# Algolzw/image-restoration-sde

Hardware: AMD Instinct MI355X
Metric: restored images/sec at 256x256, 100-step IR-SDE reverse sampler (higher is better)
Workload: dtype f32; 1 GPU; IR-SDE deraining ConditionalUNet nf=64 depth=4, reverse_sde, batch=16/GPU 256x256, T=100 (BASELINE.json configs[1]); compute_dtype=fp32, global_batch=16

## Files before the change

### image_restoration_sde_amd/_lib.py

```python
import ctypes
import os
import subprocess
import threading

_HERE = os.path.dirname(os.path.abspath(__file__))
LIB_PATH = os.environ.get("IRSDE_LIB_PATH") or os.path.join(_HERE, "libirsde_hip.so")
CSRC = os.path.join(_HERE, "csrc")

MODE = {"sde": 0, "ode": 1, "posterior": 2, "dsde_sde": 3, "dsde_ode": 4}
COEF_STRIDE = 12
FLAG_KEEP_ACTIVATIONS = 1
FLAG_NAIVE_CONV = 2
FLAG_NO_WINOGRAD = 4
FLAG_NO_WINOGRAD_F43 = 8
FLAG_UNCOND_FULLATTN = 16
FLAG_BF16 = 32
FLAG_NAF_INTRO_SKIP = 64
FLAG_BF16_ACT = 128
FLAG_NO_FUSED_LN = 256
FLAG_NAF_LENS = 512
FLAG_FP16 = 1024
FLAG_NO_WINOGRAD_FUSED = 2048
FLAG_NO_FUSED_ATTN = 4096
FLAG_NO_NAF_CHAIN = 8192
FLAG_SPLIT_BF16X2 = 16384
FLAG_SPLIT_F16X2 = 32768
FLAG_NAF_STEREO = 65536
FLAG_NAF_UNCOND = 131072
SAMPLE_GRAPH = 1
SAMPLE_PROFILE = 2

SYMBOLS = [
    "irsde_last_error", "irsde_version", "irsde_create", "irsde_create_nafnet", "irsde_destroy", "irsde_num_weights",
    "irsde_weight_name", "irsde_weight_shape", "irsde_load_weight", "irsde_finalize_weights",
    "irsde_set_schedule", "irsde_unet_forward", "irsde_sample", "irsde_sde_step", "irsde_philox_normal",
    "irsde_get_profile", "irsde_debug_tap", "irsde_work_model", "irsde_debug_conv", "irsde_plan_describe", "irsde_bench_conv", "irsde_op_profile", "irsde_debug_split_gemm", "irsde_bench_naf_chain", "irsde_debug_force_subbatches", "irsde_debug_force_chain_groups", "irsde_debug_scam",
    "irsde_eval_metrics", "irsde_tensor2img",
    "irsde_set_lens_info", "irsde_create_latent_unet", "irsde_latent_shapes", "irsde_latent_encode", "irsde_latent_decode", "irsde_latent_hidden",
]


class IrsdeLibraryError(RuntimeError):
    pass


class IrsdeError(RuntimeError):
    pass


class Config(ctypes.Structure):
    _fields_ = [("in_nc", ctypes.c_int32), ("out_nc", ctypes.c_int32), ("nf", ctypes.c_int32),
                ("depth", ctypes.c_int32), ("device", ctypes.c_int32), ("flags", ctypes.c_int32)]


class NafConfig(ctypes.Structure):
    _fields_ = [("img_channel", ctypes.c_int32), ("width", ctypes.c_int32), ("middle_blk_num", ctypes.c_int32),
                ("n_enc", ctypes.c_int32), ("enc_blk_nums", ctypes.c_int32 * 8), ("n_dec", ctypes.c_int32),
                ("dec_blk_nums", ctypes.c_int32 * 8), ("device", ctypes.c_int32), ("flags", ctypes.c_int32)]


class LatentConfig(ctypes.Structure):
    _fields_ = [("in_ch", ctypes.c_int32), ("out_ch", ctypes.c_int32), ("ch", ctypes.c_int32), ("n_mult", ctypes.c_int32),
                ("ch_mult", ctypes.c_int32 * 8), ("embed_dim", ctypes.c_int32), ("device", ctypes.c_int32),
                ("flags", ctypes.c_int32)]


_lib = None
_lock = threading.Lock()


PROBES_LIB_PATH = os.path.join(_HERE, "libirsde_hip_probes.so")


def build_library(force=False, verbose=False, probes=True):
    if force:
        subprocess.run(["make", "-C", CSRC, "clean"], check=True, capture_output=not verbose)
    for extra in ([], ["PROBES=1"]) if probes else ([],):
        r = subprocess.run(["make", "-j8", "-C", CSRC] + extra, capture_output=True, text=True)
        if r.returncode != 0:
            raise IrsdeLibraryError("building libirsde_hip%s.so failed:\n" % ("_probes" if extra else "") + r.stdout + r.stderr)
        if verbose:
            print(r.stdout)
    return LIB_PATH


def _declare(lib):
    c = ctypes
    P = c.c_void_p
    lib.irsde_last_error.restype = c.c_char_p
    lib.irsde_last_error.argtypes = []
    lib.irsde_version.restype = c.c_int
    lib.irsde_create.argtypes = [c.POINTER(Config), c.POINTER(P)]
    lib.irsde_create_nafnet.argtypes = [c.POINTER(NafConfig), c.POINTER(P)]
    lib.irsde_destroy.argtypes = [P]
    lib.irsde_destroy.restype = None
    lib.irsde_num_weights.argtypes = [P]
    lib.irsde_weight_name.argtypes = [P, c.c_int]
    lib.irsde_weight_name.restype = c.c_char_p
    lib.irsde_weight_shape.argtypes = [P, c.c_int, c.POINTER(c.c_int64), c.POINTER(c.c_int)]
    lib.irsde_load_weight.argtypes = [P, c.c_char_p, P, c.POINTER(c.c_int64), c.c_int]
    lib.irsde_finalize_weights.argtypes = [P]
    lib.irsde_set_schedule.argtypes = [P, c.c_int, P]
    lib.irsde_unet_forward.argtypes = [P, P, P, c.POINTER(c.c_int64), c.c_int, c.c_int, c.c_int, c.c_int, P, P]
    lib.irsde_sample.argtypes = [P, c.c_int, P, P, P, c.c_uint64, c.c_uint64, c.c_int, c.c_int, c.c_int,
                                 c.c_int, c.c_int, P, P, c.c_int]
    lib.irsde_sde_step.argtypes = [c.c_int, c.c_int, P, P, P, P, P, c.c_uint64, c.c_uint64, c.c_int, c.c_int,
                                   c.c_int, c.c_int, P]
    lib.irsde_philox_normal.argtypes = [P, c.c_int, c.c_int, c.c_int, c.c_uint64, c.c_uint64, P]
    lib.irsde_get_profile.argtypes = [P, c.POINTER(c.c_double)]
    lib.irsde_debug_tap.argtypes = [P, c.c_char_p, P, c.POINTER(c.c_int64)]
    lib.irsde_work_model.argtypes = [P, c.c_int, c.c_int, c.c_int, c.POINTER(c.c_double)]
    lib.irsde_debug_conv.argtypes = [P, c.c_int, P, c.c_int, c.c_int, c.c_int, c.c_int, c.c_int, P, c.c_int, c.c_int,
                                     c.c_int, c.c_int, c.c_int, P, P, c.c_int, c.c_int, P, P, c.c_int, c.c_int, P]
    lib.irsde_plan_describe.argtypes = [P, c.c_int, c.c_int, c.c_int, c.c_char_p, c.c_int]
    lib.irsde_op_profile.argtypes = [P, c.c_char_p, c.c_int]
    lib.irsde_bench_conv.argtypes = [c.c_int] * 11 + [c.POINTER(c.c_double)]
    lib.irsde_bench_naf_chain.argtypes = [c.c_int] * 4 + [c.POINTER(c.c_double)]
    lib.irsde_debug_force_subbatches.argtypes = [c.c_int]
    lib.irsde_debug_force_chain_groups.argtypes = [c.c_int]
    lib.irsde_debug_scam.argtypes = [P, c.c_int, c.c_int, c.c_int, c.c_int] + [P] * 12 + [P, P]
    lib.irsde_debug_split_gemm.argtypes = [P, P, P, c.c_int, c.c_int, c.c_int, c.c_int, c.c_int, P]
    lib.irsde_eval_metrics.argtypes = [P, P, c.c_int, c.c_int, c.c_int, c.c_int, c.c_int, c.POINTER(c.c_double), P]
    lib.irsde_tensor2img.argtypes = [P, P, c.c_int, c.c_int, c.c_int, c.c_int, P]
    lib.irsde_set_lens_info.argtypes = [P, c.POINTER(c.c_float), c.c_int]
    lib.irsde_create_latent_unet.argtypes = [c.POINTER(LatentConfig), c.POINTER(P)]
    lib.irsde_latent_shapes.argtypes = [P, c.c_int, c.c_int, c.POINTER(c.c_int64), c.POINTER(c.c_int64), c.POINTER(c.c_int)]
    lib.irsde_latent_encode.argtypes = [P, P, c.c_int, c.c_int, c.c_int, P, c.POINTER(P), P]
    lib.irsde_latent_decode.argtypes = [P, P, c.POINTER(P), c.c_int, c.c_int, c.c_int, P, P]
    lib.irsde_latent_hidden.argtypes = [P, c.c_int, c.c_int, c.c_int, c.c_int, P, P]
    for name in SYMBOLS:
        getattr(lib, name)
    return lib


def lib():
    global _lib
    with _lock:
        if _lib is None:
            if not os.path.exists(LIB_PATH):
                raise IrsdeLibraryError(
                    "libirsde_hip.so not found at %s — build it with `python -c 'import __graft_entry__ as g; "
                    "g.build()'` or `make -C %s`. There is no CPU/PyTorch fallback for this path." % (LIB_PATH, CSRC))
            try:
                _lib = _declare(ctypes.CDLL(LIB_PATH))
            except OSError as ex:
                raise IrsdeLibraryError("failed to load %s: %s" % (LIB_PATH, ex)) from ex
        return _lib


_probes = None


def probes_lib():
    global _probes
    with _lock:
        if _probes is None:
            if not os.path.exists(PROBES_LIB_PATH):
                raise IrsdeLibraryError("libirsde_hip_probes.so not found at %s — build it with `make -C %s PROBES=1`" % (PROBES_LIB_PATH, CSRC))
            try:
                _probes = _declare(ctypes.CDLL(PROBES_LIB_PATH))
            except OSError as ex:
                raise IrsdeLibraryError("failed to load %s: %s" % (PROBES_LIB_PATH, ex)) from ex
        return _probes


def check(rc, L=None):
    if rc != 0:
        msg = (L or lib()).irsde_last_error()
        raise IrsdeError("libirsde_hip error %d: %s" % (rc, msg.decode() if msg else "?"))


def stream_ptr(torch_stream=None):
    import torch
    s = torch_stream if torch_stream is not None else torch.cuda.current_stream()
    return ctypes.c_void_p(s.cuda_stream)
```

### image_restoration_sde_amd/csrc/common.h

```cpp
#pragma once
#include <hip/hip_runtime.h>
#include <cstdint>
#include <cstdio>
#include <cstdlib>
#include <stdexcept>
#include <string>
#include <vector>

namespace irsde {

struct HipError : std::runtime_error {
    using std::runtime_error::runtime_error;
};
struct HipOutOfMemory : HipError {
    using HipError::HipError;
};

inline int tuning_env_int(const char* name, int dflt) {
    static const bool on = [] { const char* t = getenv("IRSDE_TUNING"); return t && atoi(t) == 1; }();
    if (!on) return dflt;
    const char* v = getenv(name);
    return v ? atoi(v) : dflt;
}

// ... 50 lines not shown
    const float* in0 = nullptr;
    const float* in1 = nullptr;
    int C0 = 0, C1 = 0, Hin = 0, Win = 0, in_shift = 0;
    int B = 0, TH = 0, TW = 0, T = 0;
    int tile = 2;
    float* V = nullptr;
    unsigned short* Vs = nullptr;
    int nplanes = 0;
    long long v_plane = 0;
    int v_f16 = 0;
    float v_scale = 1.f;
    int v_pairs = 0;
    const float* M = nullptr;
    int Cout = 0;
    float* out = nullptr;
    int out_stride = 0;
    const float* bias = nullptr;
    const float* film = nullptr;
    int film_bstride = 0;
    int silu = 0;
    const float* res = nullptr;
    int res_stride = 0;
};
void launch_wino_input(const WinoParams& p, hipStream_t s);
struct SplitGemmArgs {
    const unsigned short* a = nullptr;
    const unsigned short* b = nullptr;
    float* out = nullptr;
    long long plA = 0, plB = 0, pA = 0, pB = 0, pO = 0;
    int M = 0, N = 0, K = 0, lda = 0, ldc = 0;
    float out_scale = 1.f;
    int n_inner = 1;
    int nblk_n = 0;
};
void gemm_split_global_init();
int gemm_split_inner(int M, int N, int ncomp);
void launch_gemm_split_pairs(const SplitGemmArgs& a, int ncomp, hipStream_t s, int abl = 0, bool f16 = false);
void launch_split_pairs(const float* in, unsigned short* out, size_t rows, int K, hipStream_t s, bool f16 = false,
                        float scale = 1.0f);
void launch_gemm_split(const SplitGemmArgs& a, int nplanes, int ncomp, hipStream_t s);
void launch_split_planes(const float* in, unsigned short* out, size_t n, size_t plane, int nplanes, hipStream_t s, bool f16 = false,
                         float scale = 1.0f);
void launch_wino_output(const WinoParams& p, hipStream_t s);
void wino_transform_weights(const float* w_packed, int Cout, int Cin, float* U, int tile);
bool wino_fused_eligible(const ConvParams& p);
void wino_fused_pack_weights(const float* U, int Cout, int Cin, float* Uf);
void launch_wino_fused(const ConvParams& p, const float* Uf, hipStream_t s, unsigned long long* dbg = nullptr, int dflags = 0);
int wino_fused_num_blocks(const ConvParams& p);
bool wino_fused64_eligible(const ConvParams& p);
void wino_fused64_pack_weights(const float* U, int Cout, int Cin, float* Uf);
void launch_wino_fused64(const ConvParams& p, const float* Uf, hipStream_t s, int variant = 0);
void wino_fused64_set_debug(unsigned long long* buf);
constexpr float kWinoFused64PairVScale = 0.0625f;
void launch_wino_fused64_split_weights(const float* Uf, unsigned short* out, size_t nfloats, float scale, hipStream_t s);
int wino_fused64_num_blocks(const ConvParams& p);
bool wino_fused64_xcd_nb(const ConvParams& p);
void wino_fused_global_init();
int device_cu_count();
bool wino_fused64t_eligible(const ConvParams& p);
long long wino_fused64t_num_items(const ConvParams& p);
void launch_wino_fused64t(const ConvParams& p, const float* Uf, hipStream_t s, int variant = 0);
void wino_fused64t_set_debug(unsigned long long* buf);
void wino_fused_t_global_init();
void naf_chain_global_init();
void naf_chain_set_debug(unsigned long long* buf);
bool naf_chain_shape_ok(int H, int W, int c);
size_t naf_chain_weight_halves(int nblocks);
size_t naf_chain_vec_floats(int nblocks);
void launch_naf_chain(const float* x, float* out, const unsigned short* w, const float* vecs, int nblocks, int B, const float* film, int film_bstride,
                      int film_off, const float* cam, int cam_bstride, int cam_off, hipStream_t s, int variant = 0);
std::vector<int> naf_chain_split_order(int nblocks, int G);
void naf_chain_build_split_weights(const unsigned short* w1, unsigned short* dst, int nblocks, int G, hipStream_t s);
size_t naf_chain_split_scratch_bytes(int B);
int naf_chain_split_groups(int B, int G);
void launch_naf_chain_split(const float* x, float* out, const unsigned short* wG, const float* vecs, int nblocks, int B, const float* film, int film_bstride,
                            int film_off, const float* cam, int cam_bstride, int cam_off, int G, void* scratch, hipStream_t s);
const unsigned* naf_chain_split_error_flag(const void* scratch, int B);
void naf_chain_split_reset(void* scratch, int B);
void naf_chain_set_sabotage(int on);
void attention_global_init();

double conv_flops(const ConvParams& p);
void launch_conv(const ConvParams& p, hipStream_t s);
void conv_global_init();
void conv_halo_global_init();
bool conv_halo_eligible(const ConvParams& p);
bool conv_halo2_wanted(const ConvParams& p, int force);
void launch_conv_halo(const ConvParams& p, hipStream_t s, int force_halo2 = 0);
void conv_set_variant(int v);
void launch_fill_random(float* p, size_t n, unsigned seed, float scale, hipStream_t s);
__device__ __forceinline__ float silu_hw(const float v) {
    return v * __builtin_amdgcn_rcpf(1.0f + __builtin_amdgcn_exp2f(v * -1.44269504088896341f));
}

void launch_f32_to_bf16(const float* in, unsigned short* out, size_t n, hipStream_t s);
void launch_f32_to_f16(const float* in, unsigned short* out, size_t n, hipStream_t s);
void launch_bf16_to_f32(const unsigned short* in, float* out, size_t n, hipStream_t s);
void launch_conv_naive(const ConvParams& p, hipStream_t s);

void launch_layernorm(const float* x, const float* g, const float* res, float* out, int64_t M, int C,
                      float eps, hipStream_t s, bool bf16 = false);
void launch_layernorm_film(const float* x, const float* g, const float* scale, const float* shift, int film_bstride,
                           int64_t pixels_per_image, float* out, int64_t M, int C, float eps, hipStream_t s);
int dwgate_tiles(int H, int W, int c);
bool naf_lnconv_ok(int c, int Cout, long long M);
void launch_naf_pwconv(const float* x, const float* in_scale, int64_t pixels_per_image, const unsigned short* w16, const float* bias, const float* ch_scale,
                       const float* res, float* out, int64_t M, int c, int Cout, hipStream_t s);
void naf_lnconv_global_init();
void launch_naf_lnconv(const float* x, const float* g, const float* fscale, const float* fshift, int film_bstride, int64_t pixels_per_image,
                       const unsigned short* w16, const float* bias, float* out, int64_t M, int c, int Cout, int gate, const float* gate_film,
                       int gate_film_bstride, hipStream_t s);
void launch_dwconv_gate(const float* u, const float* w, const float* bias, float* out, float* partial, int B, int H, int W,
                        int c, hipStream_t s);
void launch_sca(const float* partial, int ntiles, const float* W, const float* bias, float* mean, float* s_out, int B,
                int c, int HW, hipStream_t s);
void launch_row_gate(const float* in, float* out, int rows, int h, hipStream_t s);

struct AttnWorkspace {
    float* pmax = nullptr;
    float* pctx = nullptr;
    float* psum = nullptr;
    float* ctx = nullptr;
    int nch = 0;
};
int attn_num_chunks(int N, int B);
void launch_linear_attention(const float* qkv, float* out, int B, int N, const AttnWorkspace& ws, hipStream_t s,
                             bool bf16 = false);

void launch_attention_kv_context(const float* xn, const float* wkv, int B, int N, int C, const AttnWorkspace& ws, hipStream_t s,
                                 const float* ln_g = nullptr, float ln_eps = 1e-5f, const unsigned short* wkv_pair = nullptr,
                                 float w_inv_scale = 1.f, int op16 = 0, bool act_bf16 = false);
void launch_attention_q_out(const float* q, float* out, int B, int N, const AttnWorkspace& ws, hipStream_t s);
void launch_attention_q_out_fused(const float* xn, const float* x, const float* wq, const float* wout, const float* bias,
                                  const float* g2, float* y, int B, int N, int C, float eps, const AttnWorkspace& ws, hipStream_t s,
                                  const float* ln_g = nullptr, const unsigned short* wq_pair = nullptr, const unsigned short* wout_pair = nullptr,
                                  float wq_inv = 1.f, float wout_inv = 1.f, int op16 = 0, bool act_bf16 = false);

void scam_check_shape(int H, int W, int c);
void launch_scam_prologue(const float* x, const float* g_l, const float* g_r, float* xs2, int B, int H, int W, int c, hipStream_t s);
void launch_scam_core(const float* qv, float* F, int B, int H, int W, int c, hipStream_t s);
void launch_scam_epilogue(const float* x, const float* F, const float* beta, const float* gamma, float* out, int B, int H, int W, int c, hipStream_t s);
void scam_pack_proj(const float* w1, const float* b1, const float* w2, const float* b2, int c, std::vector<float>& w, std::vector<float>& bias);
void launch_stereo_prep(const float* xt, const float* cond, float* x0, int B, int ic, int P, int H, int W, int Hp, int Wp, hipStream_t s);
void launch_stereo_pack_pred(const float* in, float* out, int B, int ic, int Hp, int Wp, int in_stride, int out_stride, hipStream_t s);

void launch_full_attention(const float* qkv, float* out, int B, int N, hipStream_t s);

void launch_prep_input(const float* xt, const float* cond, float* x0, int B, int in_nc, int H, int W, int Hp, int Wp,
                       hipStream_t s, int reflect = 1);

enum Act { ACT_NONE = 0, ACT_SILU = 1, ACT_GELU = 2 };
void launch_sinusoid(const float* tvals, const float* freqs, float* out, int rows, int half, hipStream_t s);
void launch_row_linear(const float* in, int in_stride, const float* W, const float* b, float* out, int out_stride,
                       int rows, int in_dim, int out_dim, int act_in, int act_out, hipStream_t s);

struct StepState {
    int t;
    int t_next;
    int pad0, pad1;
    float coef[12];
};
void launch_step_begin(StepState* st, const float* film_table, int film_row, float* film_cur,
                       const float* coef_table, hipStream_t s);
void launch_set_step(StepState* st, int t_next, hipStream_t s);

struct SampleCtl {
    int mode;
    int pad;
    const float* noise;
    long long noise_tstride;
    unsigned long long seed;
    unsigned long long image_offset;
};
void launch_set_ctl(SampleCtl* ctl, int mode, const float* noise, long long noise_tstride, unsigned long long seed,
                    unsigned long long image_offset, hipStream_t s);

void launch_unpack_pred(const float* pred, float* out, int B, int C, int H, int W, int Hp, int Wp, int stride, hipStream_t s);
void launch_add(const float* a, const float* b, float* out, size_t n, hipStream_t s);
void launch_nchw_to_nhwc_pad(const float* in, float* out, int B, int C, int H, int W, int Hp, int Wp, int Cp, int reflect,
                             hipStream_t s);
void launch_nhwc_to_nchw(const float* in, float* out, int B, int C, int H, int W, hipStream_t s, bool bf16 = false);

struct UpdateParams {
    float* x;
    const float* mu;
    const float* pred;
    int64_t sb, sc, sy, sx;
    const float* noise;
    int64_t noise_tstride;
    const StepState* st;
    const SampleCtl* ctl;
    int t_imm;
    float coef_imm[12];
    int mode;
    int B, C, H, W;
    uint64_t seed;
    uint64_t image_offset;
    int batch0;
};
void launch_sde_update(const UpdateParams& p, hipStream_t s);
void launch_philox_normal(float* out, int B, int CHW, int t, uint64_t seed, uint64_t image_offset, hipStream_t s);

void eval_metrics(const float* out, const float* gt, int B, int C, int H, int W, int crop, double* sums_host, hipStream_t s);
void tensor2img_u8(const float* in, unsigned char* out, int B, int C, int H, int W, hipStream_t s);

}
```

### image_restoration_sde_amd/csrc/conv_igemm.hip

```cpp
#include "common.h"
#include <type_traits>
#include <mutex>
#include <vector>

namespace irsde {

typedef float floatx16 __attribute__((ext_vector_type(16)));
typedef float floatx4 __attribute__((ext_vector_type(4)));
typedef __bf16 bf16x8 __attribute__((ext_vector_type(8)));
typedef __bf16 bf16x4 __attribute__((ext_vector_type(4)));
typedef _Float16 f16x8 __attribute__((ext_vector_type(8)));
typedef _Float16 f16x4 __attribute__((ext_vector_type(4)));

namespace {

template <bool F16>
struct Op16 {
    using x8 = bf16x8;
    using x4 = bf16x4;
    static __device__ __forceinline__ floatx16 mfma(x8 a, x8 b, floatx16 c) { return __builtin_amdgcn_mfma_f32_32x32x16_bf16(a, b, c, 0, 0, 0); }
};
template <>
struct Op16<true> {
    using x8 = f16x8;
// ... 1127 lines not shown
}

}

void conv_set_variant(int v) { g_variant = v; }

int device_cu_count() {
    static std::mutex mu;
    static std::vector<int> cache;
    int dev = 0;
    IRSDE_HIP_CHECK(hipGetDevice(&dev));
    std::lock_guard<std::mutex> lk(mu);
    if ((int)cache.size() <= dev) cache.resize(dev + 1, 0);
    if (cache[dev] == 0) {
        int n = 0;
        IRSDE_HIP_CHECK(hipDeviceGetAttribute(&n, hipDeviceAttributeMultiprocessorCount, dev));
        cache[dev] = n > 0 ? n : 256;
    }
    return cache[dev];
}

void conv_global_init() {
    conv_halo_global_init();
    wino_fused_global_init();
    wino_fused_t_global_init();
    naf_chain_global_init();
    attention_global_init();
    naf_lnconv_global_init();
    gemm_split_global_init();
    IRSDE_HIP_CHECK(hipFuncSetAttribute(reinterpret_cast<const void*>(gemm_zloop_kernel<128, 128, 2, 2, 2>),
                                        hipFuncAttributeMaxDynamicSharedMemorySize, 160 * 1024));
    IRSDE_HIP_CHECK(hipFuncSetAttribute(reinterpret_cast<const void*>(gemm_zloop_kernel<128, 64, 2, 2, 2>),
                                        hipFuncAttributeMaxDynamicSharedMemorySize, 160 * 1024));
    IRSDE_HIP_CHECK(hipFuncSetAttribute(reinterpret_cast<const void*>(gemm_zloop_kernel<64, 128, 1, 4, 2>),
                                        hipFuncAttributeMaxDynamicSharedMemorySize, 160 * 1024));
    init_cfg_pair<256, 256, 2, 4, 2, false>();
    init_cfg_pair<256, 256, 2, 4, 2, true>();
    init_cfg_pair<256, 128, 4, 2, 2, false>();
    init_cfg_pair<256, 128, 4, 2, 2, true>();
    init_cfg_pair<128, 64, 2, 2, 2, false>();
    init_cfg_pair<128, 64, 2, 2, 2, true>();
    init_cfg<128, 128, 2, 2, 2, false>();
    init_cfg<128, 64, 2, 2, 2, false>();
    init_cfg<128, 32, 4, 1, 2, false>();
    init_cfg<256, 128, 4, 2, 2, false>();
    init_cfg<256, 256, 2, 4, 2, false>();
    init_cfg<128, 128, 2, 2, 2, true>();
    init_cfg<128, 64, 2, 2, 2, true>();
    init_cfg<128, 32, 4, 1, 2, true>();
    init_cfg<256, 256, 2, 4, 2, true>();
    init_cfg<128, 128, 2, 2, 2, true, false, true>();
    init_cfg<128, 64, 2, 2, 2, true, false, true>();
    init_cfg<128, 32, 4, 1, 2, true, false, true>();
    init_cfg<256, 256, 2, 4, 2, true, false, true>();
    init_cfg<128, 128, 2, 2, 2, false, true>();
    init_cfg<128, 64, 2, 2, 2, false, true>();
    init_cfg<128, 32, 4, 1, 2, false, true>();
    init_cfg<128, 128, 2, 2, 2, true, true>();
    init_cfg<128, 64, 2, 2, 2, true, true>();
    init_cfg<128, 32, 4, 1, 2, true, true>();
}

double conv_flops(const ConvParams& p) {
    return 2.0 * (double)p.B * p.Ho * p.Wo * (double)p.Cout * (double)(p.KH * p.KW) * (double)(p.C0 + p.C1);
}

bool conv_use_tile256(int M, int Cout, int splits, int nk_total) {
    if (splits != 1 || Cout % 256) return false;
    const long long nb = (long long)((M + 255) / 256) * (Cout / 256);
    return nb % 256 == 0 || nb >= 1024;
}

static int f32_narrow(const ConvParams& p, int M) {
    int bn = p.Cout >= 128 ? 128 : p.Cout > 32 ? 64 : 32;
    static const int k = tuning_env_int("IRSDE_SMALL_BN_F32", 0);
    if (k && g_variant == 0) {
        const long long slots = (long long)k * device_cu_count();
        auto blocks = [&](int n) { return (long long)((M + 127) / 128) * ((p.Cout + n - 1) / n) * p.splits * p.nz; };
        while (bn > 32 && blocks(bn) < slots) bn >>= 1;
    }
    return bn;
}

void launch_conv(const ConvParams& p, hipStream_t s) {
    const int M = p.B * p.Ho * p.Wo;
    const int Ctot = p.C0 + p.C1;
    if (p.C0 % 32 || p.C1 % 32 || Ctot == 0)
        throw HipError("launch_conv: channel counts must be multiples of 32 (got " + std::to_string(p.C0) + "+" +
                       std::to_string(p.C1) + ")");
    if (p.splits > 1 && !p.partial) throw HipError("launch_conv: split-K needs a partial buffer");
    if (p.ln_g && (p.splits != 1 || (p.Cout != 64 && p.Cout != 128) || p.nz != 1 || (p.out_stride & 3) || (p.res && (p.res_stride & 3))))
        throw HipError("launch_conv: fused LayerNorm needs Cout == 64 or 128 in one tile, no split-K");
    if (!p.zeros) throw HipError("launch_conv: ConvParams::zeros (zero page for out-of-image taps) is not set");
    if (p.w_pair) {
        if (p.w_bf || p.in_bf16 || p.out_bf16 || p.nz != 1) throw HipError("launch_conv: split-operand pairs go with fp32 storage, one component");
        if (p.in_scale && p.C1) throw HipError("launch_conv: in_scale needs a single source");
        if (p.ln_g) throw HipError("launch_conv: the fused LayerNorm epilogue (BN == Cout) is not available on the PAIR tiles");
        const int nk = p.KH * p.KW * (Ctot / 32);
        static const int t256 = tuning_env_int("IRSDE_PAIR_TILE256", 1);
        static const int inscale256 = tuning_env_int("IRSDE_PAIR_INSCALE256", 0);
        if (t256 && (!p.in_scale || inscale256) && p.Cout % 256 == 0 && (long long)((M + 255) / 256) * (p.Cout / 256) * p.splits >= 256 && g_variant != 61) {
            if (p.in_scale) launch_cfg_pair<256, 256, 2, 4, 2, true>(p, M, nk, s);
            else launch_cfg_pair<256, 256, 2, 4, 2, false>(p, M, nk, s);
        } else if (p.Cout >= 128 && M >= 256) {
            if (p.in_scale) launch_cfg_pair<256, 128, 4, 2, 2, true>(p, M, nk, s);
            else launch_cfg_pair<256, 128, 4, 2, 2, false>(p, M, nk, s);
        } else {
            if (p.in_scale) launch_cfg_pair<128, 64, 2, 2, 2, true>(p, M, nk, s);
            else launch_cfg_pair<128, 64, 2, 2, 2, false>(p, M, nk, s);
        }
        if (p.splits > 1) {
            const size_t total = (size_t)M * p.Cout;
            hipLaunchKernelGGL(conv_splitk_reduce, dim3((unsigned)((total + 255) / 256)), dim3(256), 0, s, p, M);
            IRSDE_HIP_CHECK(hipGetLastError());
        }
        return;
    }
    if (!p.w_bf && g_variant == 0 && p.Cout <= 3 && p.C0 == 64 && p.KH == 3 && p.KW == 3 && p.stride == 1 && p.pad_y == 1 && p.pad_x == 1 &&
        !p.in_shift && !p.C1 && !p.film && !p.silu && !p.res && p.splits == 1 && p.nz == 1 && !p.gate && !p.shuffle &&
        !p.ch_scale && !p.in_scale && !p.ln_g && M >= 65536) {
        hipLaunchKernelGGL(conv3x3_narrow_kernel, dim3((M + 16 * kNarrowPPG - 1) / (16 * kNarrowPPG)), dim3(256), 0, s, p, M);
        IRSDE_HIP_CHECK(hipGetLastError());
        return;
    }
    if (const int zb = zloop_batch(p)) {
        using C = Cfg<128, 128, 2, 2, false>;
        ZLoopArgs g{};
        g.a0 = p.in0; g.a1 = nullptr; g.C0 = p.C0; g.C1 = 0; g.lda0 = p.C0; g.lda1 = 0;
        g.b = p.w; g.out = p.out; g.bias = nullptr;
        g.M = p.Wo; g.N = p.Cout; g.K = p.C0; g.ldc = p.Cout;
        g.n_inner = zb; g.n_outer = 1; g.pA = p.z_in; g.pB = p.z_w; g.pO = p.z_out; g.col_step = 0; g.row_step = 0;
        g.nblk_n = (p.Cout + 127) / 128;
        if (zloop_small_m(p)) {
            using C64 = Cfg<64, 128, 1, 4, false>;
            dim3 grid64(((p.Wo + 63) / 64) * g.nblk_n, p.nz / zb);
            hipLaunchKernelGGL((gemm_zloop_kernel<64, 128, 1, 4, 2>), grid64, dim3(C64::NT), C64::MAIN_BYTES, s, g);
            IRSDE_HIP_CHECK(hipGetLastError());
            return;
        }
        if (p.Cout <= 64) {
            using C64n = Cfg<128, 64, 2, 2, false>;
            g.nblk_n = 1;
            dim3 grid_n((p.Wo + 127) / 128, p.nz / zb);
            hipLaunchKernelGGL((gemm_zloop_kernel<128, 64, 2, 2, 2>), grid_n, dim3(C64n::NT), C64n::MAIN_BYTES, s, g);
            IRSDE_HIP_CHECK(hipGetLastError());
            return;
        }
        dim3 grid(((p.Wo + 127) / 128) * g.nblk_n, p.nz / zb);
        hipLaunchKernelGGL((gemm_zloop_kernel<128, 128, 2, 2, 2>), grid, dim3(C::NT), C::MAIN_BYTES, s, g);
        IRSDE_HIP_CHECK(hipGetLastError());
        return;
    }
    if (const int mb = zloop_1x1_rows(p)) {
        using C = Cfg<128, 128, 2, 2, false>;
        const int M = p.B * p.Ho * p.Wo;
        ZLoopArgs g{};
        g.a0 = p.in0; g.a1 = p.C1 ? p.in1 : nullptr; g.C0 = p.C0; g.C1 = p.C1; g.lda0 = p.pix0; g.lda1 = p.pix1;
        g.b = p.w; g.out = p.out; g.bias = p.bias;
        g.M = M; g.N = p.Cout; g.K = p.C0 + p.C1; g.ldc = p.out_stride;
        g.n_inner = (p.Cout + 127) / 128; g.n_outer = mb; g.pA = g.pB = g.pO = 0; g.col_step = 128; g.row_step = 128;
        g.nblk_n = 1;
        const int mtiles = (M + 127) / 128;
        dim3 grid((mtiles + mb - 1) / mb, 1);
        if (p.Cout <= 64) {
            using C64n = Cfg<128, 64, 2, 2, false>;
            g.col_step = 64;
            hipLaunchKernelGGL((gemm_zloop_kernel<128, 64, 2, 2, 2>), grid, dim3(C64n::NT),
                               C64n::MAIN_BYTES + (p.bias ? 64 * 4 : 0), s, g);
            IRSDE_HIP_CHECK(hipGetLastError());
            return;
        }
        const int lds = C::MAIN_BYTES + (p.bias ? g.n_inner * 128 * 4 : 0);
        hipLaunchKernelGGL((gemm_zloop_kernel<128, 128, 2, 2, 2>), grid, dim3(C::NT), lds, s, g);
        IRSDE_HIP_CHECK(hipGetLastError());
        return;
    }
    const int nk_total = p.KH * p.KW * (Ctot / 32);
    if ((p.in_bf16 || p.out_bf16) && !p.w_bf) throw HipError("launch_conv: bf16 activation storage needs the bf16-MFMA mode");
    if (p.f16 && (!p.w_bf || p.in_bf16 || p.out_bf16)) throw HipError("launch_conv: fp16 operands go with fp32 activation storage");
    if (p.in_bf16 && (p.in_scale || p.gate || p.shuffle)) throw HipError("launch_conv: NAFNet fusions are fp32-storage only");
    if (p.in_scale) {
        if (p.C1) throw HipError("launch_conv: in_scale needs a single source");
        if (p.w_bf) {
            int bn = p.Cout >= 128 ? 128 : p.Cout > 32 ? 64 : 32;
            static const int small_bn = tuning_env_int("IRSDE_SMALL_BN", 2);
            if (small_bn && g_variant == 0) {
                const long long slots = (long long)small_bn * device_cu_count();
                auto blocks = [&](int n) { return (long long)((M + 127) / 128) * ((p.Cout + n - 1) / n) * p.splits * p.nz; };
                while (bn > 32 && blocks(bn) < slots) bn >>= 1;
            }
            if (bn == 128) launch_cfg<128, 128, 2, 2, 2, true, true>(p, M, nk_total, s);
            else if (bn == 64) launch_cfg<128, 64, 2, 2, 2, true, true>(p, M, nk_total, s);
            else launch_cfg<128, 32, 4, 1, 2, true, true>(p, M, nk_total, s);
        } else {
            if (p.Cout >= 128) launch_cfg<128, 128, 2, 2, 2, false, true>(p, M, nk_total, s);
            else if (p.Cout > 32) launch_cfg<128, 64, 2, 2, 2, false, true>(p, M, nk_total, s);
            else launch_cfg<128, 32, 4, 1, 2, false, true>(p, M, nk_total, s);
        }
    } else if (p.w_bf && g_variant != 60 && g_variant != 61 && conv_halo_eligible(p)) {
        launch_conv_halo(p, s, g_variant == 64 ? 1 : g_variant == 65 ? -1 : 0);
        return;
    } else if (p.w_bf && p.in_bf16) {
        if (p.Cout >= 128) {
            if (g_variant != 61 && (g_variant == 60 || conv_use_tile256(M, p.Cout, p.splits, nk_total)))
                launch_cfg<256, 256, 2, 4, 2, true, false, true>(p, M, nk_total, s);
// ... 57 lines not shown
```

### image_restoration_sde_amd/csrc/engine.h

```cpp
#pragma once
#include <algorithm>
#include <cmath>
#include <cstring>
#include <functional>
#include <map>
#include <memory>
#include <mutex>
#include <string>
#include <vector>

#include "../../include/irsde_hip.h"
#include "common.h"

namespace irsde {

constexpr int kWinoFusedMaxCin = 256, kWinoFusedMaxCout = 256;
inline long long wino_fused_min_tiles() { return tuning_env_int("IRSDE_WINO_FUSED_MINT", 4096); }
inline bool wino_fused64_enabled() { return tuning_env_int("IRSDE_WINO_FUSED64", 1) != 0; }
inline bool wino_fused64_pair_enabled() { return tuning_env_int("IRSDE_WINO_FUSED64_PAIR", 1) != 0; }
inline int wino_fused64_max_cin() { return tuning_env_int("IRSDE_WINO_FUSED64_MAXCIN", 512); }
inline int wino_fused64_max_cout() { return tuning_env_int("IRSDE_WINO_FUSED64_MAXCOUT", 512); }
inline long long wino_fused64_min_tiles() { return tuning_env_int("IRSDE_WINO_FUSED64_MINT", 1024); }
inline int wino_fused64t_mode() { return tuning_env_int("IRSDE_WINO_FUSED64T", 1); }
inline bool naf_lnconv_enabled() { return tuning_env_int("IRSDE_NAF_LNCONV", 1) != 0; }
// ... 100 lines not shown
    w.out.M = Mb; w.out.Cout = d.Cout; w.out.out = d.out; w.out.out_stride = d.out_stride; w.out.bias = d.bias;
    w.out.film = d.film; w.out.film_bstride = d.film_bstride; w.out.silu = d.silu; w.out.res = d.res;
    w.out.res_stride = d.res_stride;
    ConvParams& g = w.gemm;
    g.in0 = V; g.C0 = Ctot; g.pix0 = Ctot; g.Hin = 1; g.Win = T; g.w = U; g.Cout = d.Cout;
    g.KH = g.KW = 1; g.stride = 1; g.pad_y = g.pad_x = 0; g.B = 1; g.Ho = 1; g.Wo = T;
    g.out = Mb; g.out_stride = d.Cout; g.zeros = d.zeros;
    g.nz = ncomp; g.z_in = (long long)T * Ctot; g.z_w = (long long)d.Cout * Ctot; g.z_out = (long long)T * d.Cout;
    return w;
}
struct WinoSplitPlan {
    WinoParams in, out;
    SplitGemmArgs gemm;
    int nplanes = 0;
    bool f16 = false;
};
inline WinoSplitPlan make_wino_split(const ConvParams& d, const unsigned short* Us, unsigned short* Vs, float* Mb, int nplanes) {
    const WinoPlan w = make_wino(d, nullptr, nullptr, Mb, 4);
    WinoSplitPlan sp;
    sp.in = w.in; sp.out = w.out; sp.nplanes = nplanes;
    const int Ctot = d.C0 + d.C1;
    const long long T = w.in.T;
    sp.in.Vs = Vs; sp.in.nplanes = nplanes; sp.in.v_plane = 36ll * T * Ctot;
    SplitGemmArgs& g = sp.gemm;
    g.a = Vs; g.b = Us; g.out = Mb;
    g.plA = 36ll * T * Ctot; g.plB = 36ll * d.Cout * Ctot;
    g.pA = T * Ctot; g.pB = (long long)d.Cout * Ctot; g.pO = T * d.Cout;
    g.M = (int)T; g.N = d.Cout; g.K = Ctot; g.lda = Ctot; g.ldc = d.Cout;
    g.n_inner = gemm_split_inner(g.M, g.N, 36);
    return sp;
}
constexpr float kSplitF16VScale = 1.0f / 16.0f;
inline WinoSplitPlan make_wino_pairs(const ConvParams& d, const unsigned short* Up, unsigned short* Vs, float* Mb, bool f16 = false,
                                     float u_scale = 1.f) {
    const WinoPlan w = make_wino(d, nullptr, nullptr, Mb, 4);
    WinoSplitPlan sp;
    sp.in = w.in; sp.out = w.out; sp.nplanes = 2;
    const int Ctot = d.C0 + d.C1;
    const long long T = w.in.T;
    sp.in.Vs = Vs; sp.in.nplanes = 2; sp.in.v_pairs = 1;
    sp.in.v_f16 = f16 ? 1 : 0; sp.in.v_scale = f16 ? kSplitF16VScale : 1.f;
    SplitGemmArgs& g = sp.gemm;
    g.out_scale = f16 ? 1.0f / (kSplitF16VScale * u_scale) : 1.f;
    sp.f16 = f16;
    g.a = Vs; g.b = Up; g.out = Mb;
    g.pA = T * Ctot; g.pB = (long long)d.Cout * Ctot; g.pO = T * d.Cout;
    g.M = (int)T; g.N = d.Cout; g.K = Ctot; g.lda = Ctot; g.ldc = d.Cout;
    return sp;
}
inline int split_min_cin() { return tuning_env_int("IRSDE_SPLIT_MINC", 256); }
inline int split_direct_min_k() { return tuning_env_int("IRSDE_SPLIT_DIRECT_MINK", 128); }
inline bool wino_shape_ok(const ConvParams& d, int tile) {
    return d.KH == 3 && d.KW == 3 && d.stride == 1 && d.pad_y == 1 && d.pad_x == 1 && d.Ho % tile == 0 && d.Wo % tile == 0 &&
           (d.C0 + d.C1) % 32 == 0 && d.Cout % 4 == 0 && d.out_stride % 4 == 0 && (!d.res || d.res_stride % 4 == 0);
}

inline float pow2_scale_into_512(const float* host, size_t n) {
    float mx = 0.f;
    for (size_t i = 0; i < n; ++i) mx = std::max(mx, std::fabs(host[i]));
    return mx > 0.f ? std::exp2(std::floor(std::log2(512.0f / mx))) : 1.f;
}

struct Tensor {
    float* p = nullptr;
    int B = 0, H = 0, W = 0, C = 0;
    bool bf16 = false;
    size_t numel() const { return (size_t)B * H * W * C; }
};

struct PoolBlock {
    float* p;
    size_t n;
    bool free;
};

struct Plan {
    int B = 0, H = 0, W = 0, Hp = 0, Wp = 0;
    bool per_sample_film = false;
    StepState* own_step = nullptr;
    float* own_film = nullptr;
    int slot = 0, b0 = 0;
    std::vector<PoolBlock> pool;
    std::vector<Op> net_ops;
    float* xin = nullptr;
    float* cin = nullptr;
    float* x0 = nullptr;
    float* pred = nullptr;
    int pred_stride = 4;
    std::map<std::string, Tensor> taps;
    hipGraphExec_t graph_exec = nullptr;
    hipGraph_t graph = nullptr;
    double conv_flops = 0, conv_bytes = 0, conv_exec_flops = 0;
    uint64_t last_use = 0;
    std::vector<std::pair<void*, int>> chain_scratch;
    std::vector<const unsigned*> chain_err;

    ~Plan() {
        if (graph_exec) (void)hipGraphExecDestroy(graph_exec);
        if (graph) (void)hipGraphDestroy(graph);
        for (auto& b : pool) (void)hipFree(b.p);
    }
    float* alloc(size_t n, bool reuse) {
        if (reuse) {
            int best = -1;
            for (int i = 0; i < (int)pool.size(); ++i)
                if (pool[i].free && pool[i].n >= n && (best < 0 || pool[i].n < pool[best].n)) best = i;
            if (best >= 0 && pool[best].n <= n + n / 2 + 1024) {
                pool[best].free = false;
                return pool[best].p;
            }
        }
        float* p = nullptr;
        const hipError_t err = hipMalloc(&p, std::max<size_t>(n, 64) * sizeof(float));
        if (err == hipErrorOutOfMemory) {
            (void)hipGetLastError();
            throw HipOutOfMemory("plan arena: hipMalloc of " + std::to_string(std::max<size_t>(n, 64) * sizeof(float)) + " bytes failed (out of memory)");
        }
        IRSDE_HIP_CHECK(err);
        pool.push_back({p, n, false});
        return p;
    }
    void release(float* p) {
        for (auto& b : pool)
            if (b.p == p) {
                b.free = true;
                return;
            }
    }
};

struct LatentPlan {
    bool decode = false;
    std::unique_ptr<Plan> plan;
    Tensor image;
    Tensor latent;
    std::vector<Tensor> hidden;
    std::vector<int> hidden_c;
    bool resident = false;
};

}

using namespace irsde;

struct irsde_engine {
    irsde_config cfg{};
    int time_dim = 0;
    std::vector<std::string> names;
    std::map<std::string, HostTensor> host;
    bool finalized = false;
    std::vector<float*> dev_allocs;

    ConvW init_conv, final_conv;
    float *tm_w1 = nullptr, *tm_b1 = nullptr, *tm_w3 = nullptr, *tm_b3 = nullptr, *freqs = nullptr;
    std::vector<ResW> down_res;
    std::vector<AttnW> down_attn;
    std::vector<ConvW> down_conv;
    ResW mid1, mid2;
    AttnW mid_attn;
    std::vector<ResW> up_res;
    std::vector<AttnW> up_attn;
    std::vector<ConvW> up_conv;
    ResW final_res;
    std::vector<ResW*> all_res;
    int film_row = 0;

    int arch = 0;
    int naf_ic = 0;
    std::vector<int> naf_enc_nums, naf_dec_nums;
    int naf_mid_num = 0;
    std::vector<std::vector<NafBlockW>> naf_enc, naf_dec;
    std::vector<NafBlockW> naf_mid;
    std::vector<ConvW> naf_downs, naf_ups;
    ConvW naf_intro, naf_ending;
    std::vector<NafBlockW*> naf_all;
    std::vector<NafChainW> naf_chain_enc, naf_chain_dec;
    NafChainW naf_chain_mid;
    float *cm_w1 = nullptr, *cm_b1 = nullptr, *cm_w3 = nullptr, *cm_b3 = nullptr;
    int cam_row = 0;
    float* cam_cur = nullptr;
    int cam_rows = 0;
    int cam_set = 0;

    int lat_in = 0, lat_out = 0, lat_ch = 0, lat_embed = 0;
    std::vector<int> lat_mult;
    ConvW lat_init, lat_latent, lat_post, lat_final;
    std::vector<ResW> lat_enc_res, lat_dec_res;
    AttnW lat_enc_attn, lat_dec_attn;
    std::vector<ConvW> lat_down, lat_up;
    std::vector<std::unique_ptr<LatentPlan>> lat_plans;

    int T = 0;
    float* coef_table = nullptr;
    float* film_table = nullptr;
    float* film_cur = nullptr;
    int film_cur_rows = 0;
    StepState* step = nullptr;
    SampleCtl* ctl = nullptr;

    float* zeros = nullptr;
    hipStream_t stream = nullptr;
    hipEvent_t ev_in = nullptr, ev_out = nullptr;
    static constexpr int kMaxSub = 4;
    hipStream_t sub_stream[kMaxSub - 1] = {nullptr, nullptr, nullptr};
    hipEvent_t ev_fork = nullptr, ev_join[kMaxSub - 1] = {nullptr, nullptr, nullptr};
    std::vector<std::unique_ptr<Plan>> plans;
    uint64_t use_counter = 0;
    double profile[12] = {0};
    std::vector<double> op_ms;
    std::vector<std::string> op_desc;
    int op_steps = 0;
    int plan_parts = 1;
    int op_split = 1;
    std::vector<hipEvent_t> ev_pool;
    std::mutex mu;

    float* dmalloc(size_t n) {
        float* p = nullptr;
        IRSDE_HIP_CHECK(hipMalloc(&p, std::max<size_t>(n, 16) * sizeof(float)));
        dev_allocs.push_back(p);
        return p;
    }
    std::map<const float*, unsigned short*> bf16_copies;
    const unsigned short* bf16_copy(const float* w, size_t n) {
        auto it = bf16_copies.find(w);
        if (it != bf16_copies.end()) return it->second;
        unsigned short* d = nullptr;
        IRSDE_HIP_CHECK(hipMalloc(&d, n * sizeof(unsigned short)));
        if (cfg.flags & IRSDE_FLAG_FP16) launch_f32_to_f16(w, d, n, stream);
        else launch_f32_to_bf16(w, d, n, stream);
        IRSDE_HIP_CHECK(hipStreamSynchronize(stream));
        bf16_copies[w] = d;
        return d;
    }
    struct PairCopy { unsigned short* p; float inv_scale; };
    std::map<const float*, PairCopy> pair_copies;
    PairCopy pair_copy(const float* w, size_t n) {
        return make_pair_copy(pair_copies, w, n, [&](unsigned short* d, bool f16, float sc) { launch_split_planes(w, d, n, n, 2, stream, f16, sc); });
    }
    std::map<const float*, PairCopy> pair_copies_il;
    PairCopy pair_copy_il(const float* w, size_t rows, int K) {
        return make_pair_copy(pair_copies_il, w, rows * (size_t)K, [&](unsigned short* d, bool f16, float sc) { launch_split_pairs(w, d, rows, K, stream, f16, sc); });
    }
    template <class Split>
    PairCopy make_pair_copy(std::map<const float*, PairCopy>& cache, const float* w, size_t n, Split split) {
        auto it = cache.find(w);
        if (it != cache.end()) return it->second;
        const bool f16 = (cfg.flags & IRSDE_FLAG_SPLIT_F16X2) != 0;
        float sc = 1.f;
        if (f16) {
            std::vector<float> h(n);
            IRSDE_HIP_CHECK(hipMemcpy(h.data(), w, n * sizeof(float), hipMemcpyDeviceToHost));
            sc = pow2_scale_into_512(h.data(), n);
        }
        unsigned short* d = nullptr;
        IRSDE_HIP_CHECK(hipMalloc(&d, 2 * n * sizeof(unsigned short)));
        dev_allocs.push_back(reinterpret_cast<float*>(d));
        split(d, f16, sc);
        IRSDE_HIP_CHECK(hipStreamSynchronize(stream));
        const PairCopy pc{d, 1.0f / sc};
        cache[w] = pc;
        return pc;
    }
    float* upload(const std::vector<float>& v) {
        float* p = dmalloc(v.size());
        IRSDE_HIP_CHECK(hipMemcpy(p, v.data(), v.size() * sizeof(float), hipMemcpyHostToDevice));
        return p;
    }
};

namespace irsde {

inline bool naf_lens(const irsde_engine* e) { return (e->cfg.flags & IRSDE_FLAG_NAF_LENS) != 0; }
inline bool naf_stereo(const irsde_engine* e) { return e->arch == 1 && (e->cfg.flags & IRSDE_FLAG_NAF_STEREO) != 0; }
inline bool uncond_engine(const irsde_engine* e) {
    return (e->arch == 0 && (e->cfg.flags & IRSDE_FLAG_UNCOND_FULLATTN) != 0) || (e->arch == 1 && (e->cfg.flags & IRSDE_FLAG_NAF_UNCOND) != 0);
}
inline int rup32(int c) { return (c + 31) & ~31; }
inline StepState* step_of(const irsde_engine* e, const Plan* pl) { return pl->own_step ? pl->own_step : e->step; }
inline float* film_of(const irsde_engine* e, const Plan* pl) { return pl->own_film ? pl->own_film : e->film_cur; }

void build_inventory(irsde_engine* e);
void build_inventory_naf(irsde_engine* e);
void build_inventory_latent(irsde_engine* e);
void finalize(irsde_engine* e);
void compute_film_rows(irsde_engine* e, const float* tvals, int rows, float* dst, hipStream_t s);
void ensure_film_cur(irsde_engine* e, int rows);

Plan* get_plan(irsde_engine* e, int B, int H, int W, bool per_sample_film, int slot = 0, int b0 = 0);
int naf_subbatches(const irsde_engine* e, int B, int H, int W);
void set_force_chain_groups(int g);
int forced_chain_groups();
void set_force_subbatches(int n);
LatentPlan* get_latent_plan(irsde_engine* e, int B, int H, int W, bool decode);

int guard(const std::function<void()>& f);

}
```

### image_restoration_sde_amd/csrc/engine_api.hip

```cpp
#include "engine.h"
#include <cmath>

using namespace irsde;

namespace irsde {
namespace {

thread_local std::string g_last_error;

hipEvent_t get_event(irsde_engine* e, size_t i) {
    while (e->ev_pool.size() <= i) {
        hipEvent_t ev;
        IRSDE_HIP_CHECK(hipEventCreate(&ev));
        e->ev_pool.push_back(ev);
    }
    return e->ev_pool[i];
}

void run_net(Plan* pl, hipStream_t s) {
    for (auto& op : pl->net_ops) op.fn(s);
}

UpdateParams make_update(irsde_engine* e, Plan* pl) {
    UpdateParams u{};
    u.x = pl->xin; u.mu = pl->cin; u.pred = pl->pred;
    const int64_t ps = pl->pred_stride;
    u.sb = (int64_t)pl->Hp * pl->Wp * ps; u.sc = 1; u.sy = (int64_t)pl->Wp * ps; u.sx = ps;
    u.st = step_of(e, pl); u.ctl = e->ctl;
    u.B = pl->B; u.C = e->cfg.in_nc; u.H = pl->H; u.W = pl->W;
    u.batch0 = pl->b0;
    return u;
}

void one_step(irsde_engine* e, Plan* pl, hipStream_t s) {
    launch_step_begin(step_of(e, pl), e->film_table, e->film_row, film_of(e, pl), e->coef_table, s);
    run_net(pl, s);
    launch_sde_update(make_update(e, pl), s);
}

void ensure_step_graph(irsde_engine* e, Plan* pl, hipStream_t s) {
    if (pl->graph_exec) return;
    IRSDE_HIP_CHECK(hipStreamBeginCapture(s, hipStreamCaptureModeThreadLocal));
    try {
        one_step(e, pl, s);
    } catch (...) {
        hipGraph_t g = nullptr;
        (void)hipStreamEndCapture(s, &g);
        if (g) (void)hipGraphDestroy(g);
        throw;
    }
    IRSDE_HIP_CHECK(hipStreamEndCapture(s, &pl->graph));
    IRSDE_HIP_CHECK(hipGraphInstantiate(&pl->graph_exec, pl->graph, nullptr, nullptr, 0));
}

void ensure_sub_streams(irsde_engine* e, int n) {
    if (!e->ev_fork) IRSDE_HIP_CHECK(hipEventCreateWithFlags(&e->ev_fork, hipEventDisableTiming));
    for (int i = 0; i + 1 < n; ++i) {
        if (!e->sub_stream[i]) IRSDE_HIP_CHECK(hipStreamCreateWithFlags(&e->sub_stream[i], hipStreamNonBlocking));
        if (!e->ev_join[i]) IRSDE_HIP_CHECK(hipEventCreateWithFlags(&e->ev_join[i], hipEventDisableTiming));
    }
}

void apply_fp16_flag(irsde_engine* e) {
    if (!(e->cfg.flags & IRSDE_FLAG_FP16)) return;
    if (e->cfg.flags & IRSDE_FLAG_BF16_ACT) {
        delete e;
        throw HipError("IRSDE_FLAG_FP16 keeps fp32 activation storage: it cannot be combined with IRSDE_FLAG_BF16_ACT");
    }
    e->cfg.flags |= IRSDE_FLAG_BF16;
}

}

int guard(const std::function<void()>& f) {
    try {
        f();
        return IRSDE_OK;
    } catch (const HipError& ex) {
        g_last_error = ex.what();
        const std::string m = ex.what();
        if (m.find("weight") != std::string::npos) return IRSDE_ERR_WEIGHT;
        if (m.find(" failed: ") != std::string::npos) return IRSDE_ERR_HIP;
        return IRSDE_ERR_INVALID;
    } catch (const std::exception& ex) {
        g_last_error = ex.what();
        return IRSDE_ERR_INVALID;
    }
}

}

extern "C" {

const char* irsde_last_error(void) { return g_last_error.c_str(); }
int irsde_version(void) { return 107; }

int irsde_create(const irsde_config* cfg, irsde_engine** out) {
    return guard([&] {
        if (!cfg || !out) throw HipError("null argument");
        if (cfg->nf % 32 || cfg->nf < 32) throw HipError("nf must be a positive multiple of 32");
        if (cfg->depth < 1 || cfg->depth > 6) throw HipError("depth out of range");
        if (cfg->in_nc < 1 || cfg->in_nc > 4 || cfg->out_nc < 1 || cfg->out_nc > 4)
            throw HipError("in_nc/out_nc must be in 1..4");
        if (cfg->in_nc != cfg->out_nc) throw HipError("sampler needs in_nc == out_nc");
        if ((cfg->nf << cfg->depth) > 2048) throw HipError("nf * 2^depth must be <= 2048");
        if (cfg->flags & IRSDE_FLAG_NAF_STEREO) throw HipError("IRSDE_FLAG_NAF_STEREO: the stereo network is a ConditionalNAFNet (irsde_create_nafnet)");
        if (cfg->flags & IRSDE_FLAG_NAF_UNCOND) throw HipError("IRSDE_FLAG_NAF_UNCOND: irsde_create_nafnet only (the unconditional UNet is IRSDE_FLAG_UNCOND_FULLATTN)");
        auto* e = new irsde_engine();
        e->cfg = *cfg;
        if (cfg->flags & IRSDE_FLAG_BF16_ACT) {
            if (cfg->flags & (IRSDE_FLAG_UNCOND_FULLATTN | IRSDE_FLAG_NAIVE_CONV)) {
                delete e;
                throw HipError("IRSDE_FLAG_BF16_ACT: only the conditional UNet on the MFMA kernels stores bf16 activations");
            }
            e->cfg.flags |= IRSDE_FLAG_BF16;
        }
        apply_fp16_flag(e);
        e->time_dim = cfg->nf * 4;
        build_inventory(e);
        *out = e;
// ... 152 lines not shown
        IRSDE_HIP_CHECK(hipMemcpyAsync(pl->xin, xt, img, hipMemcpyDeviceToDevice, s));
        if (cond) IRSDE_HIP_CHECK(hipMemcpyAsync(pl->cin, cond, img, hipMemcpyDeviceToDevice, s));
        const bool in_table = nt == 1 && e->film_table && t_host[0] >= 0 && t_host[0] <= e->T;
        if (in_table) {
            IRSDE_HIP_CHECK(hipMemcpyAsync(e->film_cur, e->film_table + (size_t)t_host[0] * e->film_row,
                                           (size_t)e->film_row * 4, hipMemcpyDeviceToDevice, s));
        } else {
            const int rows = (naf_stereo(e) && nt > 1 ? 2 : 1) * nt;
            std::vector<float> tv(rows);
            for (int i = 0; i < rows; ++i) tv[i] = (float)t_host[i % nt];
            float* dtv = nullptr;
            IRSDE_HIP_CHECK(hipMalloc(&dtv, rows * sizeof(float)));
            IRSDE_HIP_CHECK(hipMemcpy(dtv, tv.data(), rows * sizeof(float), hipMemcpyHostToDevice));
            compute_film_rows(e, dtv, rows, e->film_cur, s);
            (void)hipFree(dtv);
        }
        run_net(pl, s);
        launch_unpack_pred(pl->pred, out, B, e->cfg.out_nc, H, W, pl->Hp, pl->Wp, pl->pred_stride, s);
        IRSDE_HIP_CHECK(hipEventRecord(e->ev_out, s));
        IRSDE_HIP_CHECK(hipStreamWaitEvent(user, e->ev_out, 0));
    });
}

int irsde_sample(irsde_engine* e, int mode, const float* xT, const float* mu, const float* noise, uint64_t seed,
                 uint64_t image_offset, int B, int H, int W, int T, int t_stop, float* out, void* stream,
                 int flags) {
    return guard([&] {
        if (!e || !xT || !out) throw HipError("null argument");
        if (!e->finalized || !e->film_table) throw HipError("sample: weights/schedule not set");
        if (mode < 0 || mode > 4) throw HipError("sample: bad mode");
        const bool uncond_e = uncond_engine(e);
        if ((mode >= 3) != uncond_e) throw HipError("sample: DenoisingSDE modes (3,4) go with the unconditional network and vice versa");
        if (!mu && !uncond_e) throw HipError("null argument");
        if (T < 0) T = e->T;
        if (T > e->T) throw HipError("sample: T exceeds the schedule length");
        if (B < 1 || H < 2 || W < 2) throw HipError("sample: bad shape");
        if (t_stop < 0 || (T > 0 && t_stop >= T) || (T == 0 && t_stop != 0)) throw HipError("sample: t_stop must be in [0, T)");
        const int nsteps = T - t_stop;
        std::lock_guard<std::mutex> lk(e->mu);
        DeviceScope dev_scope(e->cfg.device);
        hipStream_t user = reinterpret_cast<hipStream_t>(stream);
        if (T == 0) {
            IRSDE_HIP_CHECK(hipMemcpyAsync(out, xT, (size_t)B * e->cfg.in_nc * H * W * 4, hipMemcpyDeviceToDevice, user));
            return;
        }
        hipStream_t s = e->stream;
        const bool profile = (flags & IRSDE_SAMPLE_PROFILE) != 0;
        const bool graph = (flags & IRSDE_SAMPLE_GRAPH) != 0 && !profile;
        const size_t img = (size_t)B * e->cfg.in_nc * H * W;
        for (auto& p : e->plans)
            for (const unsigned* f : p->chain_err) {
                unsigned v = 0;
                IRSDE_HIP_CHECK(hipMemcpy(&v, f, 4, hipMemcpyDeviceToHost));
                if (v) {
                    for (auto& sc : p->chain_scratch) naf_chain_split_reset(sc.first, sc.second);
                    char code[32];
                    snprintf(code, sizeof code, " [flag 0x%x]", v);
                    throw HipError(std::string("sample: the previous call's split NAFBlock-chain kernel timed out waiting for a work-group that was not resident (its results were invalid); "
                                               "set IRSDE_TUNING=1 IRSDE_NAF_CHAIN_SPLIT=1 if other work shares this GPU") + code);
                }
            }
        const int nsub = profile ? 1 : naf_subbatches(e, B, H, W);
        const int Bs = B / nsub;
        const size_t simg = img / nsub;
        struct Part { Plan* pl; hipStream_t st; };
        std::vector<Part> parts(nsub);
        auto part_plan = [&](int i) { return get_plan(e, Bs, H, W, false, nsub > 1 ? i + 1 : 0, i * Bs); };
        struct PartsScope { irsde_engine* e; PartsScope(irsde_engine* e_, int n) : e(e_) { e->plan_parts = n; } ~PartsScope() { e->plan_parts = 1; } } parts_scope(e, nsub);
        for (int i = 0; i < nsub; ++i) parts[i].pl = part_plan(i);
        for (int i = 0; i < nsub; ++i) (void)part_plan(i);
        if (nsub > 1) ensure_sub_streams(e, nsub);
        for (int i = 0; i < nsub; ++i) parts[i].st = i == 0 ? s : e->sub_stream[i - 1];
        IRSDE_HIP_CHECK(hipEventRecord(e->ev_in, user));
        IRSDE_HIP_CHECK(hipStreamWaitEvent(s, e->ev_in, 0));
        launch_set_ctl(e->ctl, mode, noise, (long long)img, seed, image_offset, s);
        if (nsub > 1) IRSDE_HIP_CHECK(hipEventRecord(e->ev_fork, s));
        for (int i = 0; i < nsub; ++i) {
            Plan* pl = parts[i].pl;
            hipStream_t t = parts[i].st;
            if (i > 0) IRSDE_HIP_CHECK(hipStreamWaitEvent(t, e->ev_fork, 0));
            IRSDE_HIP_CHECK(hipMemcpyAsync(pl->xin, xT + i * simg, simg * 4, hipMemcpyDeviceToDevice, t));
            if (mu) IRSDE_HIP_CHECK(hipMemcpyAsync(pl->cin, mu + i * simg, simg * 4, hipMemcpyDeviceToDevice, t));
            launch_set_step(step_of(e, pl), T, t);
            if (graph) ensure_step_graph(e, pl, t);
        }
        if (!profile) {
            for (int k = 0; k < nsteps; ++k)
                for (auto& p : parts) {
                    if (graph) IRSDE_HIP_CHECK(hipGraphLaunch(p.pl->graph_exec, p.st));
                    else one_step(e, p.pl, p.st);
                }
        } else {
            Plan* pl = parts[0].pl;
            std::vector<int> kinds;
            size_t ei = 0;
            auto mark = [&](int kind) {
                IRSDE_HIP_CHECK(hipEventRecord(get_event(e, ei++), s));
                kinds.push_back(kind);
            };
            for (int i = 0; i < nsteps; ++i) {
                mark(OP_OTHER);
                launch_step_begin(step_of(e, pl), e->film_table, e->film_row, film_of(e, pl), e->coef_table, s);
                for (auto& op : pl->net_ops) {
                    mark(op.kind);
                    op.fn(s);
                }
                mark(OP_OTHER);
                launch_sde_update(make_update(e, pl), s);
            }
            IRSDE_HIP_CHECK(hipEventRecord(get_event(e, ei++), s));
            IRSDE_HIP_CHECK(hipStreamSynchronize(s));
            double ms[OP_NKINDS] = {0, 0, 0, 0, 0};
            const size_t per_step = pl->net_ops.size() + 2;
            e->op_ms.assign(pl->net_ops.size(), 0.0);
            e->op_desc.clear();
            for (auto& op : pl->net_ops) e->op_desc.push_back(op.desc);
            e->op_steps = nsteps;
            e->op_split = naf_subbatches(e, B, H, W);
            for (size_t k = 0; k < kinds.size(); ++k) {
                float t;
                IRSDE_HIP_CHECK(hipEventElapsedTime(&t, e->ev_pool[k], e->ev_pool[k + 1]));
                ms[kinds[k]] += t;
                const size_t in_step = k % per_step;
                if (in_step >= 1 && in_step <= pl->net_ops.size()) e->op_ms[in_step - 1] += t;
            }
            hipEvent_t e0 = e->ev_pool[0], e1 = e->ev_pool[kinds.size()];
            float wall;
            IRSDE_HIP_CHECK(hipEventElapsedTime(&wall, e0, e1));
            size_t nconv = 0;
            for (auto& op : pl->net_ops) nconv += op.kind == OP_CONV;
            e->profile[0] = ms[OP_CONV];
            e->profile[1] = pl->conv_flops * nsteps;
            e->profile[2] = (double)nconv * nsteps;
            e->profile[3] = pl->conv_bytes * nsteps;
            e->profile[4] = ms[OP_LN];
            e->profile[5] = ms[OP_ATTN];
            e->profile[6] = ms[OP_OTHER];
            e->profile[7] = wall;
            e->profile[8] = nsteps;
            e->profile[9] = ms[OP_WINO];
            e->profile[10] = pl->conv_exec_flops * nsteps;
            e->profile[11] = 0;
        }
        for (int i = 0; i < nsub; ++i) {
            IRSDE_HIP_CHECK(hipMemcpyAsync(out + i * simg, parts[i].pl->xin, simg * 4, hipMemcpyDeviceToDevice, parts[i].st));
            if (i > 0) {
                IRSDE_HIP_CHECK(hipEventRecord(e->ev_join[i - 1], parts[i].st));
                IRSDE_HIP_CHECK(hipStreamWaitEvent(s, e->ev_join[i - 1], 0));
            }
        }
        IRSDE_HIP_CHECK(hipEventRecord(e->ev_out, s));
        IRSDE_HIP_CHECK(hipStreamWaitEvent(user, e->ev_out, 0));
    });
}

int irsde_sde_step(int mode, int t, const float* coef_row, float* x, const float* mu, const float* eps_hat,
                   const float* noise_t, uint64_t seed, uint64_t image_offset, int B, int C, int H, int W,
                   void* stream) {
    return guard([&] {
        if (!coef_row || !x || !eps_hat || (!mu && mode < 3)) throw HipError("null argument");
        if (!mu) mu = x;
        if (mode < 0 || mode > 4) throw HipError("sde_step: bad mode");
        UpdateParams u{};
        u.x = x; u.mu = mu; u.pred = eps_hat;
        u.sb = (int64_t)C * H * W; u.sc = (int64_t)H * W; u.sy = W; u.sx = 1;
        u.noise = noise_t; u.noise_tstride = 0;
        u.st = nullptr; u.ctl = nullptr; u.t_imm = t;
        for (int i = 0; i < IRSDE_COEF_STRIDE; ++i) u.coef_imm[i] = coef_row[i];
        u.mode = mode; u.B = B; u.C = C; u.H = H; u.W = W; u.seed = seed; u.image_offset = image_offset;
        launch_sde_update(u, reinterpret_cast<hipStream_t>(stream));
    });
}

int irsde_philox_normal(float* out, int B, int CHW, int t, uint64_t seed, uint64_t image_offset, void* stream) {
    return guard([&] {
        if (!out) throw HipError("null argument");
        launch_philox_normal(out, B, CHW, t, seed, image_offset, reinterpret_cast<hipStream_t>(stream));
    });
}

int irsde_get_profile(const irsde_engine* e, double out[12]) {
    if (!e || !out) return IRSDE_ERR_INVALID;
    for (int i = 0; i < 12; ++i) out[i] = e->profile[i];
    return IRSDE_OK;
}

int irsde_debug_tap(irsde_engine* e, const char* name, float* dst, int64_t dims[4]) {
    return guard([&] {
        if (!e || !name || !dims) throw HipError("null argument");
        if (!(e->cfg.flags & IRSDE_FLAG_KEEP_ACTIVATIONS)) throw HipError("debug_tap needs IRSDE_FLAG_KEEP_ACTIVATIONS");
        Plan* pl = nullptr;
        for (auto& p : e->plans)
            if (!pl || p->last_use > pl->last_use) pl = p.get();
        if (!pl) throw HipError("debug_tap: no forward has run");
        auto it = pl->taps.find(name);
        if (it == pl->taps.end()) throw HipError(std::string("debug_tap: unknown tap ") + name);
        const Tensor& t = it->second;
        dims[0] = t.B; dims[1] = t.C; dims[2] = t.H; dims[3] = t.W;
        if (!dst) return;
        DeviceScope dev_scope(e->cfg.device);
        IRSDE_HIP_CHECK(hipDeviceSynchronize());
        float* tmp = nullptr;
        IRSDE_HIP_CHECK(hipMalloc(&tmp, t.numel() * 4));
        launch_nhwc_to_nchw(t.p, tmp, t.B, t.C, t.H, t.W, e->stream, t.bf16);
        IRSDE_HIP_CHECK(hipStreamSynchronize(e->stream));
        IRSDE_HIP_CHECK(hipMemcpy(dst, tmp, t.numel() * 4, hipMemcpyDeviceToHost));
        (void)hipFree(tmp);
    });
}

int irsde_op_profile(irsde_engine* e, char* buf, int buflen) {
    return guard([&] {
        if (!e || !buf || buflen < 1) throw HipError("null argument");
        std::string out;
        char line[512];
        for (size_t i = 0; i < e->op_ms.size(); ++i) {
            snprintf(line, sizeof line, "%9.4f ms  %s\n", e->op_ms[i] / std::max(e->op_steps, 1), e->op_desc[i].c_str());
            out += line;
        }
        if (e->op_split > 1) {
            snprintf(line, sizeof line, "note: the un-split plan; irsde_sample runs this batch as %d concurrent sub-batches (own plans, streams, step graphs)\n", e->op_split);
            out += line;
        }
        strncpy(buf, out.c_str(), buflen - 1);
        buf[buflen - 1] = 0;
    });
}

int irsde_plan_describe(irsde_engine* e, int B, int H, int W, char* buf, int buflen) {
    return guard([&] {
        if (!e || !buf || buflen < 1) throw HipError("null argument");
        if (!e->finalized) throw HipError("plan_describe: weights not finalized");
        std::lock_guard<std::mutex> lk(e->mu);
        DeviceScope dev_scope(e->cfg.device);
        Plan* pl = get_plan(e, B, H, W, false);
        std::string out;
        for (auto& op : pl->net_ops) out += op.desc + "\n";
        const int nsub = naf_subbatches(e, B, H, W);
        if (nsub > 1) out += "note: the un-split plan; irsde_sample runs this batch as " + std::to_string(nsub) + " concurrent sub-batches of " + std::to_string(B / nsub) + " images (own plans)\n";
        strncpy(buf, out.c_str(), buflen - 1);
        buf[buflen - 1] = 0;
    });
}

int irsde_work_model(irsde_engine* e, int B, int H, int W, double out[2]) {
    return guard([&] {
        if (!e || !out) throw HipError("null argument");
        if (!e->finalized) throw HipError("work_model: weights not finalized");
        std::lock_guard<std::mutex> lk(e->mu);
        DeviceScope dev_scope(e->cfg.device);
        Plan* pl = get_plan(e, B, H, W, false);
        out[0] = pl->conv_flops;
        out[1] = pl->conv_bytes;
    });
}

int irsde_create_latent_unet(const irsde_latent_unet_config* cfg, irsde_engine** out) {
    return guard([&] {
        if (!cfg || !out) throw HipError("null argument");
        if (cfg->in_ch < 1 || cfg->in_ch > 32 || cfg->out_ch < 1 || cfg->out_ch > 4) throw HipError("in_ch must be in 1..32 and out_ch in 1..4");
        if (cfg->ch < 1 || cfg->n_mult < 1 || cfg->n_mult > 6) throw HipError("ch / ch_mult out of range");
        if (cfg->embed_dim < 1 || cfg->embed_dim > 32) throw HipError("embed_dim must be in 1..32");
        if (cfg->flags & IRSDE_FLAG_BF16_ACT) throw HipError("IRSDE_FLAG_BF16_ACT: conditional UNet only");
        auto* e = new irsde_engine();
        e->arch = 2;
        e->cfg.in_nc = cfg->in_ch; e->cfg.out_nc = cfg->out_ch; e->cfg.nf = cfg->ch; e->cfg.depth = cfg->n_mult;
        e->cfg.device = cfg->device; e->cfg.flags = cfg->flags;
        apply_fp16_flag(e);
        e->lat_in = cfg->in_ch; e->lat_out = cfg->out_ch; e->lat_ch = cfg->ch; e->lat_embed = cfg->embed_dim;
        for (int i = 0; i < cfg->n_mult; ++i) {
            if (cfg->ch_mult[i] < 1 || cfg->ch * cfg->ch_mult[i] > 2048) throw HipError("ch * ch_mult out of range");
            e->lat_mult.push_back(cfg->ch_mult[i]);
        }
        build_inventory_latent(e);
        *out = e;
    });
}

int irsde_latent_shapes(irsde_engine* e, int H, int W, int64_t latent_chw[3], int64_t* hidden_chw, int* n_hidden) {
    return guard([&] {
        if (!e || e->arch != 2 || !latent_chw || !n_hidden) throw HipError("latent_shapes: not a latent UNet engine / null argument");
        const int depth = (int)e->lat_mult.size(), sdiv = 1 << depth;
        const int Hp = (H + sdiv - 1) / sdiv * sdiv, Wp = (W + sdiv - 1) / sdiv * sdiv;
        latent_chw[0] = e->lat_embed; latent_chw[1] = Hp >> (depth - 1); latent_chw[2] = Wp >> (depth - 1);
        *n_hidden = 2 * depth + 1;
        if (hidden_chw) {
            auto dim = [&](int i) { return i == 0 ? e->lat_ch : e->lat_ch * e->lat_mult[i - 1]; };
            for (int k = 0; k < 2 * depth + 1; ++k) {
                const int lvl = k == 0 ? 0 : (k - 1) / 2;
                hidden_chw[3 * k] = dim(lvl); hidden_chw[3 * k + 1] = Hp >> lvl; hidden_chw[3 * k + 2] = Wp >> lvl;
            }
        }
    });
}

int irsde_latent_encode(irsde_engine* e, const float* x, int B, int H, int W, float* latent, float* const* hidden,
                        void* stream) {
    return guard([&] {
        if (!e || e->arch != 2 || !x || !latent) throw HipError("latent_encode: not a latent UNet engine / null argument");
        if (!e->finalized) throw HipError("latent_encode: weights not finalized");
        if (B < 1 || H < 2 || W < 2) throw HipError("latent_encode: bad shape");
        std::lock_guard<std::mutex> lk(e->mu);
        DeviceScope dev_scope(e->cfg.device);
        hipStream_t user = reinterpret_cast<hipStream_t>(stream), s = e->stream;
        LatentPlan* lp = get_latent_plan(e, B, H, W, false);
        Plan* pl = lp->plan.get();
        IRSDE_HIP_CHECK(hipEventRecord(e->ev_in, user));
        IRSDE_HIP_CHECK(hipStreamWaitEvent(s, e->ev_in, 0));
        launch_nchw_to_nhwc_pad(x, lp->image.p, B, e->lat_in, H, W, pl->Hp, pl->Wp, lp->image.C, 1, s);
        run_net(pl, s);
        const Tensor& L = lp->latent;
        launch_unpack_pred(L.p, latent, B, e->lat_embed, L.H, L.W, L.H, L.W, L.C, s);
        lp->resident = true;
        for (size_t k = 0; hidden && k < lp->hidden.size(); ++k) {
            const Tensor& h = lp->hidden[k];
            if (!hidden[k]) throw HipError("latent_encode: null hidden pointer");
            launch_unpack_pred(h.p, hidden[k], B, lp->hidden_c[k], h.H, h.W, h.H, h.W, h.C, s);
        }
        IRSDE_HIP_CHECK(hipEventRecord(e->ev_out, s));
        IRSDE_HIP_CHECK(hipStreamWaitEvent(user, e->ev_out, 0));
    });
}

int irsde_latent_decode(irsde_engine* e, const float* latent, const float* const* hidden, int B, int H, int W, float* out,
                        void* stream) {
    return guard([&] {
        if (!e || e->arch != 2 || !latent || !out) throw HipError("latent_decode: not a latent UNet engine / null argument");
        if (!e->finalized) throw HipError("latent_decode: weights not finalized");
        std::lock_guard<std::mutex> lk(e->mu);
        DeviceScope dev_scope(e->cfg.device);
        hipStream_t user = reinterpret_cast<hipStream_t>(stream), s = e->stream;
        if (!hidden) {
            bool res = false;
            for (auto& q : e->lat_plans)
                if (!q->decode && q->plan->B == B && q->plan->H == H && q->plan->W == W) res = q->resident;
            if (!res) throw HipError("latent_decode: hidden == NULL needs a preceding irsde_latent_encode of the same B x H x W on this engine");
// ... 108 lines not shown
```

### image_restoration_sde_amd/csrc/engine_debug.hip

```cpp
#include "engine.h"
#include "../../include/irsde_hip_debug.h"

using namespace irsde;

namespace irsde {
namespace {

struct Scratch {
    hipStream_t s;
    std::vector<void*> bufs;
    explicit Scratch(hipStream_t s_) : s(s_) {}
    ~Scratch() {
        (void)hipStreamSynchronize(s);
        for (void* p : bufs) (void)hipFree(p);
    }
    Scratch(const Scratch&) = delete;
    Scratch& operator=(const Scratch&) = delete;
    template <class T> T* alloc(size_t n) {
        void* p = nullptr;
        IRSDE_HIP_CHECK(hipMalloc(&p, n * sizeof(T)));
        bufs.push_back(p);
        return static_cast<T*>(p);
    }
    float* upload(const float* host, size_t n) {
// ... 18 lines not shown
    }
    ~EventPair() {
        if (e0) (void)hipEventDestroy(e0);
        if (e1) (void)hipEventDestroy(e1);
    }
    EventPair(const EventPair&) = delete;
    EventPair& operator=(const EventPair&) = delete;
};
template <class Run>
double time_launches(hipStream_t s, int iters, Run&& run) {
    EventPair ev;
    IRSDE_HIP_CHECK(hipEventRecord(ev.e0, s));
    for (int i = 0; i < iters; ++i) run();
    IRSDE_HIP_CHECK(hipEventRecord(ev.e1, s));
    IRSDE_HIP_CHECK(hipStreamSynchronize(s));
    float ms = 0.f;
    IRSDE_HIP_CHECK(hipEventElapsedTime(&ms, ev.e0, ev.e1));
    return ms / iters;
}

struct VariantScope {
    explicit VariantScope(int v) { conv_set_variant(v); }
    ~VariantScope() { conv_set_variant(0); }
};

bool code_in(const std::initializer_list<int>& codes, int c) { return std::find(codes.begin(), codes.end(), c) != codes.end(); }
bool debug_conv_code_known(int c) {
    return code_in({0, 1, 2, 3, 4, 5, 12, 13, 22, 23, 33, 34, 35, 36, 37, 42, 43, 44, 45, 46, 47, 55, 56, 62, 63, 204, 260, 261, 262, 263}, c) ||
           code_in({100, 103, 105, 106, 107, 150, 160, 161, 162, 163, 165, 166, 167, 170, 171, 172, 173}, c);
}
bool bench_conv_variant_known(int v) {
    return code_in({0, 3, 5, 6, 7, 50, 60, 61, 62, 63, 64, 65, 66, 67, 70, 71, 72, 73}, v) ||
           code_in({80, 81, 82, 412, 413, 421, 422, 423, 430, 431, 432, 434, 435, 460, 461, 462, 465, 467, 468, 469, 480, 481, 482}, v) ||
           code_in({2001, 2002, 2004, 4650, 4651, 4652, 4653}, v) ||
           (v >= 83 && v <= 82 + 255) ||
           (v >= 472 && v <= 476);
}

}
}

extern "C" {

int irsde_debug_scam(const float* x, int B, int H, int W, int C, const float* norm_l_g, const float* norm_r_g, const float* l_proj1_w,
                     const float* l_proj1_b, const float* r_proj1_w, const float* r_proj1_b, const float* l_proj2_w, const float* l_proj2_b,
                     const float* r_proj2_w, const float* r_proj2_b, const float* beta, const float* gamma, float* out, void* stream) {
    return guard([&] {
        if (!x || !out || !norm_l_g || !norm_r_g || !l_proj1_w || !l_proj1_b || !r_proj1_w || !r_proj1_b || !l_proj2_w || !l_proj2_b || !r_proj2_w ||
            !r_proj2_b || !beta || !gamma)
            throw HipError("null argument");
        if (B < 1) throw HipError("debug_scam: bad shape");
        scam_check_shape(H, W, C);
        hipStream_t s = reinterpret_cast<hipStream_t>(stream);
        conv_global_init();
        const int Hs = H / 4, Ws = W / 4;
        std::vector<float> wl, bl, wr, br;
        scam_pack_proj(l_proj1_w, l_proj1_b, l_proj2_w, l_proj2_b, C, wl, bl);
        scam_pack_proj(r_proj1_w, r_proj1_b, r_proj2_w, r_proj2_b, C, wr, br);
        Scratch mem(s);
        auto up = [&](const float* h, size_t n) {
            float* d = mem.alloc<float>(std::max<size_t>(n, 16));
            if (h) IRSDE_HIP_CHECK(hipMemcpy(d, h, n * 4, hipMemcpyHostToDevice));
            return d;
        };
        float *dgl = up(norm_l_g, C), *dgr = up(norm_r_g, C), *dbe = up(beta, C), *dga = up(gamma, C);
        float *dwl = up(wl.data(), wl.size()), *dbl = up(bl.data(), bl.size()), *dwr = up(wr.data(), wr.size()), *dbr = up(br.data(), br.size());
        const size_t vsz = (size_t)B * Hs * Ws * 2 * C;
        float *xs2 = up(nullptr, 2 * vsz), *qv = up(nullptr, 2 * vsz), *F = up(nullptr, vsz), *dz = up(nullptr, 256);
        IRSDE_HIP_CHECK(hipMemset(dz, 0, 1024));
        launch_scam_prologue(x, dgl, dgr, xs2, B, H, W, C, s);
        for (int v = 0; v < 2; ++v) {
            ConvParams p;
            p.in0 = xs2 + v * vsz; p.C0 = 2 * C; p.pix0 = 2 * C;
            p.Hin = Hs; p.Win = Ws;
            p.w = v ? dwr : dwl; p.Cout = 2 * C; p.KH = p.KW = 1; p.stride = 1;
            p.B = B; p.Ho = Hs; p.Wo = Ws;
            p.out = qv + v * vsz; p.out_stride = 2 * C;
            p.bias = v ? dbr : dbl;
            p.zeros = dz;
            launch_conv(p, s);
        }
        launch_scam_core(qv, F, B, H, W, C, s);
        launch_scam_epilogue(x, F, dbe, dga, out, B, H, W, C, s);
        IRSDE_HIP_CHECK(hipStreamSynchronize(s));
    });
}

int irsde_debug_conv(const float* in0, int C0, const float* in1, int C1, int B, int Hin, int Win, int in_shift,
                     const float* w_oihw, int Cout, int KH, int KW, int stride, int pad, const float* bias,
                     const float* film, int film_bstride, int silu, const float* res, float* out, int naive,
                     int splits, void* stream) {
    return guard([&] {
        if (!in0 || !w_oihw || !out) throw HipError("null argument");
        if (!debug_conv_code_known(naive)) throw HipError("debug_conv: unknown selector code " + std::to_string(naive));
        hipStream_t s = reinterpret_cast<hipStream_t>(stream);
        conv_global_init();
        const int Cin = C0 + C1;
        std::vector<float> pk((size_t)Cout * KH * KW * Cin);
        for (int o = 0; o < Cout; ++o)
            for (int i = 0; i < Cin; ++i)
                for (int ky = 0; ky < KH; ++ky)
                    for (int kx = 0; kx < KW; ++kx)
                        pk[(((size_t)o * KH + ky) * KW + kx) * Cin + i] = w_oihw[(((size_t)o * Cin + i) * KH + ky) * KW + kx];
        Scratch mem(s);
        float* dw = mem.upload(pk);
        float* db = bias ? mem.upload(bias, Cout) : nullptr;
        ConvParams p;
        p.in0 = in0; p.C0 = C0; p.pix0 = C0; p.in1 = in1; p.C1 = C1; p.pix1 = C1;
        p.Hin = Hin; p.Win = Win; p.in_shift = in_shift;
        p.w = dw; p.Cout = Cout; p.KH = KH; p.KW = KW; p.stride = stride; p.pad_y = pad; p.pad_x = pad;
        p.B = B;
        p.Ho = ((Hin << in_shift) + 2 * pad - KH) / stride + 1;
        p.Wo = ((Win << in_shift) + 2 * pad - KW) / stride + 1;
        p.out = out; p.out_stride = Cout; p.bias = db; p.film = film; p.film_bstride = film_bstride; p.silu = silu;
        p.res = res; p.res_stride = Cout;
        float* dz = mem.alloc<float>(256);
        IRSDE_HIP_CHECK(hipMemset(dz, 0, 1024));
        p.zeros = dz;
        const int wino_tile = (naive == 2 || naive == 12 || naive == 22) ? 2 : (naive == 3 || naive == 13 || naive == 23) ? 4 : 0;
        if (splits > 1 && naive != 1 && !wino_tile) {
            p.splits = splits;
            p.partial = mem.alloc<float>((size_t)splits * B * p.Ho * p.Wo * Cout);
        }
        if (naive == 44 || naive == 45) {
            const bool f16 = naive == 44;
            if (!wino_shape_ok(p, 4) || Cin % 32) throw HipError("debug_conv: shape not eligible for the pair GEMM");
            std::vector<float> U((size_t)36 * Cout * Cin);
            wino_transform_weights(pk.data(), Cout, Cin, U.data(), 4);
            const float us = f16 ? pow2_scale_into_512(U.data(), U.size()) : 1.f;
            const long long T = (long long)B * (p.Ho / 4) * (p.Wo / 4);
            float* dU = mem.upload(U);
            unsigned short* dUp = mem.alloc<unsigned short>(2 * U.size());
            unsigned short* dVp = mem.alloc<unsigned short>((size_t)36 * T * Cin * 2);
            float* dM = mem.alloc<float>((size_t)36 * T * Cout);
            launch_split_pairs(dU, dUp, (size_t)36 * Cout, Cin, s, f16, us);
            const WinoSplitPlan sp = make_wino_pairs(p, dUp, dVp, dM, f16, us);
            launch_wino_input(sp.in, s);
            launch_gemm_split_pairs(sp.gemm, 36, s, 0, f16);
            launch_wino_output(sp.out, s);
        } else if (naive == 42 || naive == 43) {
            const int npl = naive - 40;
            if (!wino_shape_ok(p, 4)) throw HipError("debug_conv: shape not eligible for Winograd");
            std::vector<float> U((size_t)36 * Cout * Cin);
            wino_transform_weights(pk.data(), Cout, Cin, U.data(), 4);
            const long long T = (long long)B * (p.Ho / 4) * (p.Wo / 4);
            float* dU = mem.upload(U);
            unsigned short* dUs = mem.alloc<unsigned short>(U.size() * npl);
            unsigned short* dVs = mem.alloc<unsigned short>((size_t)36 * T * Cin * npl);
            float* dM = mem.alloc<float>((size_t)36 * T * Cout);
            launch_split_planes(dU, dUs, U.size(), U.size(), npl, s);
            const WinoSplitPlan sp = make_wino_split(p, dUs, dVs, dM, npl);
            launch_wino_input(sp.in, s);
            launch_gemm_split(sp.gemm, npl, 36, s);
            launch_wino_output(sp.out, s);
        } else if (naive == 35 || naive == 37 || naive == 56) {
            if (!wino_fused64_eligible(p)) throw HipError("debug_conv: shape not eligible for the fused Winograd kernel");
            std::vector<float> U((size_t)36 * Cout * Cin), Uf((size_t)36 * Cout * Cin);
            wino_transform_weights(pk.data(), Cout, Cin, U.data(), 4);
            wino_fused64_pack_weights(U.data(), Cout, Cin, Uf.data());
            const float usc = pow2_scale_into_512(U.data(), U.size());
            float* dUf = mem.upload(Uf);
            unsigned short* dUp = mem.alloc<unsigned short>(2 * Uf.size());
            launch_wino_fused64_split_weights(dUf, dUp, Uf.size(), usc, s);
            p.pair_scale = 1.0f / (kWinoFused64PairVScale * usc);
            launch_wino_fused64(p, reinterpret_cast<const float*>(dUp), s, naive == 56 ? 24 : naive == 37 ? 4 + 64 : 4);
        } else if (naive == 33 || naive == 34 || naive == 36 || naive == 55 || naive == 62 || naive == 63) {
// ... 458 lines not shown
```

### image_restoration_sde_amd/csrc/engine_plan.hip

```cpp
#include "engine.h"
#include <atomic>

using namespace irsde;

namespace irsde {

struct Builder {
    irsde_engine* e;
    Plan* pl;
    bool reuse;
    bool naive;
    int film_bstride;
    int b0 = 0;
    const float* film_base() const { return film_of(e, pl) + (size_t)b0 * film_bstride; }
    const float* cam_base() const { return e->cam_cur + (size_t)b0 * e->cam_row; }
    const float* fused_ln_g = nullptr;

    bool act_bf16() const { return (e->cfg.flags & IRSDE_FLAG_BF16_ACT) != 0; }
    Tensor talloc(int B, int H, int W, int C, int force_f32 = 0) {
        Tensor t;
        t.B = B; t.H = H; t.W = W; t.C = C;
        t.bf16 = act_bf16() && !force_f32;
        t.p = pl->alloc(t.bf16 ? (t.numel() + 1) / 2 : t.numel(), reuse);
        return t;
// ... 789 lines not shown
    for (size_t i = 1; i < e->plans.size(); ++i)
        if (e->plans[i]->last_use < e->plans[lru]->last_use) lru = i;
    IRSDE_HIP_CHECK(hipDeviceSynchronize());
    const int vb = e->plans[lru]->B, vh = e->plans[lru]->H, vw = e->plans[lru]->W;
    const bool split = e->plans[lru]->slot > 0;
    for (size_t i = e->plans.size(); i-- > 0;)
        if (i == lru || (split && e->plans[i]->slot > 0 && e->plans[i]->B == vb && e->plans[i]->H == vh && e->plans[i]->W == vw))
            e->plans.erase(e->plans.begin() + i);
    return true;
}

static Plan* build_plan(irsde_engine* e, int B, int H, int W, bool per_sample_film, int slot, int b0);

Plan* get_plan(irsde_engine* e, int B, int H, int W, bool per_sample_film, int slot, int b0) {
    for (auto& p : e->plans)
        if (p->B == B && p->H == H && p->W == W && p->per_sample_film == per_sample_film && p->slot == slot && p->b0 == b0) {
            p->last_use = ++e->use_counter;
            return p.get();
        }
    if (e->plans.size() >= 8) evict_lru_plan(e);
    for (;;) {
        try {
            return build_plan(e, B, H, W, per_sample_film, slot, b0);
        } catch (const HipOutOfMemory&) {
            if (!evict_lru_plan(e)) throw;
        }
    }
}

static Plan* build_plan(irsde_engine* e, int B, int H, int W, bool per_sample_film, int slot, int b0) {
    const bool stereo = naf_stereo(e);
    ensure_film_cur(e, per_sample_film ? (stereo ? 2 : 1) * (b0 + B) : 1);
    if (naf_lens(e)) {
        if (e->cam_set < b0 + B) throw HipError("latent-bokeh ConditionalNAFNet: irsde_set_lens_info must cover the batch first");
        if (e->cam_rows < b0 + B) throw HipError("internal: lens table smaller than the batch");
    }

    const int depth = e->cfg.depth, nf = e->cfg.nf, in_nc = e->cfg.in_nc;
    const int sdiv = 1 << depth;
    std::unique_ptr<Plan> plan(new Plan());
    Plan* pl = plan.get();
    pl->B = B; pl->H = H; pl->W = W;
    pl->Hp = (H + sdiv - 1) / sdiv * sdiv;
    pl->Wp = (W + sdiv - 1) / sdiv * sdiv;
    pl->per_sample_film = per_sample_film;
    pl->slot = slot; pl->b0 = b0;
    pl->pred_stride = (e->cfg.out_nc + 3) & ~3;
    pl->last_use = ++e->use_counter;
    if (e->arch != 1 && (pl->Hp - H >= H || pl->Wp - W >= W)) throw HipError("image too small for reflect padding");

    if (slot > 0) {
        if (per_sample_film) throw HipError("internal: sub-batch plans are sampler plans (one time step for the whole part)");
        pl->own_film = pl->alloc((size_t)e->film_row + 64, false);
        pl->own_step = reinterpret_cast<StepState*>(pl->alloc(sizeof(StepState) / 4 + 4, false));
        IRSDE_HIP_CHECK(hipMemset(pl->own_step, 0, sizeof(StepState)));
    }
    const size_t img = (size_t)B * in_nc * H * W;
    pl->xin = pl->alloc(img, false);
    pl->cin = pl->alloc(img, false);
    const bool uncond = uncond_engine(e);
    const int P = ((uncond ? 1 : 2) * (stereo ? e->naf_ic : in_nc) + 3) & ~3;
    const size_t x0n = (size_t)(stereo ? 2 * B : B) * (pl->Hp + 6) * (pl->Wp + 6) * P + 64;
    pl->x0 = pl->alloc(x0n, false);
    IRSDE_HIP_CHECK(hipMemset(pl->x0, 0, x0n * sizeof(float)));

    Builder b{e, pl, (e->cfg.flags & IRSDE_FLAG_KEEP_ACTIVATIONS) == 0, (e->cfg.flags & IRSDE_FLAG_NAIVE_CONV) != 0,
              per_sample_film ? e->film_row : 0, b0};
    {
        const float *xi = pl->xin, *ci = uncond ? nullptr : pl->cin;
        float* x0 = pl->x0;
        const int Hp = pl->Hp, Wp = pl->Wp;
        const int reflect = e->arch == 1 ? 0 : 1;
        if (stereo) {
            const int ic = e->naf_ic;
            b.push_other(OP_OTHER, [=](hipStream_t s) { launch_stereo_prep(xi, ci, x0, B, ic, P, H, W, Hp, Wp, s); });
        } else
        b.push_other(OP_OTHER, [=](hipStream_t s) { launch_prep_input(xi, ci, x0, B, in_nc, H, W, Hp, Wp, s, reflect); });
    }
    if (e->arch == 1) {
        build_naf_plan(e, pl, b, P);
        e->plans.push_back(std::move(plan));
        return pl;
    }
    Tensor x;
    {
        ConvParams p;
        p.in0 = pl->x0; p.C0 = e->init_conv.Cin; p.pix0 = P;
        p.Hin = pl->Hp + 6; p.Win = pl->Wp + 6;
        p.w = e->init_conv.w; p.Cout = nf; p.KH = 7; p.KW = 1; p.stride = 1; p.pad_y = 0; p.pad_x = 0;
        p.B = B; p.Ho = pl->Hp; p.Wo = pl->Wp;
        x = b.talloc(B, pl->Hp, pl->Wp, nf);
        p.out = x.p; p.out_stride = nf; p.out_bf16 = x.bf16;
        b.push_conv(p);
        const double real = 2.0 * (double)B * pl->Hp * pl->Wp * nf * 49.0 * ((uncond ? 1.0 : 2.0) * in_nc);
        pl->conv_flops += real - pl->net_ops.back().flops;
        pl->net_ops.back().flops = real;
    }
    b.tap("init_conv", x);
    Tensor x_init = x;
    std::vector<Tensor> hs;
    for (int i = 0; i < depth; ++i) {
        const std::string d = "downs." + std::to_string(i) + ".";
        Tensor a = b.resblock(e->down_res[2 * i], x, nullptr);
        if (x.p != x_init.p) b.tfree(x);
        b.tap(d + "0", a);
        hs.push_back(a);
        Tensor c = b.resblock(e->down_res[2 * i + 1], a, nullptr);
        b.tap(d + "1", c);
        Tensor g = b.attn(e->down_attn[i], c);
        b.tfree(c);
        b.tap(d + "2", g);
        hs.push_back(g);
        if (i != depth - 1)
            x = b.conv(e->down_conv[i], g, nullptr, 2, 1, 0, nullptr, 0, nullptr);
        else
            x = b.conv(e->down_conv[i], g, nullptr, 1, 1, 0, nullptr, 0, nullptr);
        b.tap(d + "3", x);
    }
    {
        Tensor a = b.resblock(e->mid1, x, nullptr);
        b.tfree(x);
        b.tap("mid_block1", a);
        Tensor g = b.attn(e->mid_attn, a);
        b.tfree(a);
        b.tap("mid_attn", g);
        x = b.resblock(e->mid2, g, nullptr);
        b.tfree(g);
        b.tap("mid_block2", x);
    }
    for (int j = 0; j < depth; ++j) {
        const std::string u = "ups." + std::to_string(j) + ".";
        Tensor s1 = hs.back(); hs.pop_back();
        Tensor a = b.resblock(e->up_res[2 * j], x, &s1);
        b.tfree(x); b.tfree(s1);
        b.tap(u + "0", a);
        Tensor s2 = hs.back(); hs.pop_back();
        Tensor c = b.resblock(e->up_res[2 * j + 1], a, &s2);
        b.tfree(a); b.tfree(s2);
        b.tap(u + "1", c);
        Tensor g = b.attn(e->up_attn[j], c);
        b.tfree(c);
        b.tap(u + "2", g);
        if (j != depth - 1)
            x = b.conv(e->up_conv[j], g, nullptr, 1, 1, 1, nullptr, 0, nullptr);
        else
            x = b.conv(e->up_conv[j], g, nullptr, 1, 1, 0, nullptr, 0, nullptr);
        b.tfree(g);
        b.tap(u + "3", x);
    }
    {
        Tensor f = b.resblock(e->final_res, x, &x_init);
        b.tfree(x); b.tfree(x_init);
        b.tap("final_res_block", f);
        Tensor pr = b.conv(e->final_conv, f, nullptr, 1, 1, 0, nullptr, 0, nullptr, pl->pred_stride);
        b.tfree(f);
        pl->pred = pr.p;
    }
    e->plans.push_back(std::move(plan));
    return pl;
}

LatentPlan* get_latent_plan(irsde_engine* e, int B, int H, int W, bool decode) {
    for (auto& lp : e->lat_plans)
        if (lp->decode == decode && lp->plan->B == B && lp->plan->H == H && lp->plan->W == W) {
            lp->plan->last_use = ++e->use_counter;
            return lp.get();
        }
    LatentPlan* enc = decode ? get_latent_plan(e, B, H, W, false) : nullptr;
    size_t n_shapes = 0;
    bool shape_known = false;
    for (size_t i = 0; i < e->lat_plans.size(); ++i) {
        const Plan* q = e->lat_plans[i]->plan.get();
        bool first = true;
        for (size_t j = 0; j < i; ++j) {
            const Plan* r = e->lat_plans[j]->plan.get();
            if (r->B == q->B && r->H == q->H && r->W == q->W) { first = false; break; }
        }
        n_shapes += first ? 1 : 0;
        if (q->B == B && q->H == H && q->W == W) shape_known = true;
    }
    if (!shape_known && n_shapes >= 4) {
        size_t lru = e->lat_plans.size();
        for (size_t i = 0; i < e->lat_plans.size(); ++i) {
            if (e->lat_plans[i].get() == enc) continue;
            if (lru == e->lat_plans.size() || e->lat_plans[i]->plan->last_use < e->lat_plans[lru]->plan->last_use) lru = i;
        }
        IRSDE_HIP_CHECK(hipDeviceSynchronize());
        const int vb = e->lat_plans[lru]->plan->B, vh = e->lat_plans[lru]->plan->H, vw = e->lat_plans[lru]->plan->W;
        for (size_t i = e->lat_plans.size(); i-- > 0;)
            if (e->lat_plans[i].get() != enc && e->lat_plans[i]->plan->B == vb && e->lat_plans[i]->plan->H == vh && e->lat_plans[i]->plan->W == vw)
                e->lat_plans.erase(e->lat_plans.begin() + i);
    }
    const int depth = (int)e->lat_mult.size(), ch = e->lat_ch;
    auto dim = [&](int i) { return i == 0 ? ch : ch * e->lat_mult[i - 1]; };
    const int sdiv = 1 << depth;
    std::unique_ptr<LatentPlan> lp(new LatentPlan());
    lp->decode = decode;
    lp->plan.reset(new Plan());
    Plan* pl = lp->plan.get();
    pl->B = B; pl->H = H; pl->W = W;
    pl->Hp = (H + sdiv - 1) / sdiv * sdiv;
    pl->Wp = (W + sdiv - 1) / sdiv * sdiv;
    pl->last_use = ++e->use_counter;
    if (pl->Hp - H >= H || pl->Wp - W >= W) throw HipError("image too small for reflect padding");
    Builder b{e, pl, false, (e->cfg.flags & IRSDE_FLAG_NAIVE_CONV) != 0, 0};
    std::vector<std::pair<int, int>> hgeo;
    hgeo.push_back({0, ch});
    for (int i = 0; i < depth; ++i) {
        hgeo.push_back({i, dim(i)});
        hgeo.push_back({i, dim(i)});
    }
    const int hl = pl->Hp >> (depth - 1), wl = pl->Wp >> (depth - 1);
    if (!decode) {
        lp->image = b.talloc(B, pl->Hp, pl->Wp, rup32(e->lat_in));
        Tensor x = b.conv(e->lat_init, lp->image, nullptr, 1, 1, 0, nullptr, 0, nullptr);
        lp->hidden.push_back(x);
        for (int i = 0; i < depth; ++i) {
            Tensor a = b.resblock(e->lat_enc_res[2 * i], x, nullptr);
            lp->hidden.push_back(a);
            Tensor c = b.resblock(e->lat_enc_res[2 * i + 1], a, nullptr);
            Tensor g = i == depth - 1 ? b.attn(e->lat_enc_attn, c) : c;
            lp->hidden.push_back(g);
            x = i != depth - 1 ? b.conv(e->lat_down[i], g, nullptr, 2, 1, 0, nullptr, 0, nullptr)
                               : b.conv(e->lat_down[i], g, nullptr, 1, 1, 0, nullptr, 0, nullptr);
        }
        lp->latent = b.conv(e->lat_latent, x, nullptr, 1, 0, 0, nullptr, 0, nullptr);
    } else {
        lp->latent = b.talloc(B, hl, wl, rup32(e->lat_embed));
        lp->hidden = enc->hidden;
        for (size_t k = 0; k < hgeo.size(); ++k)
            if (lp->hidden[k].H != (pl->Hp >> hgeo[k].first) || lp->hidden[k].W != (pl->Wp >> hgeo[k].first) || lp->hidden[k].C != rup32(hgeo[k].second))
                throw HipError("latent plan: encode / decode skip geometry mismatch");
        Tensor x = b.conv(e->lat_post, lp->latent, nullptr, 1, 0, 0, nullptr, 0, nullptr);
        const int nh = (int)lp->hidden.size();
        for (int j = 0; j < depth; ++j) {
            Tensor a = b.resblock(e->lat_dec_res[2 * j], x, &lp->hidden[nh - (2 * j + 1)]);
            Tensor c = b.resblock(e->lat_dec_res[2 * j + 1], a, &lp->hidden[nh - (2 * j + 2)]);
            Tensor g = j == 0 ? b.attn(e->lat_dec_attn, c) : c;
            x = j != depth - 1 ? b.conv(e->lat_up[j], g, nullptr, 1, 1, 1, nullptr, 0, nullptr)
                               : b.conv(e->lat_up[j], g, nullptr, 1, 1, 0, nullptr, 0, nullptr);
        }
        Tensor y = b.talloc(x.B, x.H, x.W, x.C);
// ... 15 lines not shown
```

### image_restoration_sde_amd/csrc/engine_weights.hip

```cpp
#include "engine.h"
#include <cmath>

using namespace irsde;

namespace irsde {

void finalize_common(irsde_engine* e);
void add_w(irsde_engine* e, const std::string& name, std::vector<int64_t> shape) {
    e->names.push_back(name);
    HostTensor t;
    t.shape = std::move(shape);
    e->host[name] = std::move(t);
}
void inv_resblock(irsde_engine* e, const std::string& p, int ci, int co) {
    const int td = e->time_dim;
    add_w(e, p + "mlp.1.weight", {2 * co, td});
    add_w(e, p + "mlp.1.bias", {2 * co});
    add_w(e, p + "block1.proj.weight", {co, ci, 3, 3});
    add_w(e, p + "block2.proj.weight", {co, co, 3, 3});
    if (ci != co) add_w(e, p + "res_conv.weight", {co, ci, 1, 1});
}
void inv_attn(irsde_engine* e, const std::string& p, int c) {
    add_w(e, p + "fn.norm.g", {1, c, 1, 1});
    add_w(e, p + "fn.fn.to_qkv.weight", {384, c, 1, 1});
// ... 47 lines not shown
    add_w(e, "final_conv.weight", {e->cfg.out_nc, nf, 3, 3});
    add_w(e, "final_conv.bias", {e->cfg.out_nc});
}

const HostTensor& need(irsde_engine* e, const std::string& n) {
    auto it = e->host.find(n);
    if (it == e->host.end() || !it->second.loaded) throw HipError("missing weight: " + n);
    return it->second;
}

ConvW pack_conv(irsde_engine* e, const std::string& wname, const std::string& bname) {
    const HostTensor& t = need(e, wname);
    const int O = (int)t.shape[0], I = (int)t.shape[1], KH = (int)t.shape[2], KW = (int)t.shape[3];
    std::vector<float> p((size_t)O * KH * KW * I);
    for (int o = 0; o < O; ++o)
        for (int i = 0; i < I; ++i)
            for (int ky = 0; ky < KH; ++ky)
                for (int kx = 0; kx < KW; ++kx)
                    p[(((size_t)o * KH + ky) * KW + kx) * I + i] = t.data[(((size_t)o * I + i) * KH + ky) * KW + kx];
    ConvW c;
    c.w = e->upload(p);
    c.Cout = O; c.Cin = I; c.KH = KH; c.KW = KW;
    if (!bname.empty()) c.bias = e->upload(need(e, bname).data);
    if (KH == 3 && KW == 3 && I % 32 == 0 && !(e->cfg.flags & (IRSDE_FLAG_NO_WINOGRAD | IRSDE_FLAG_BF16))) {
        for (int tile : {2, 4}) {
            if (tile == 4 && (e->cfg.flags & IRSDE_FLAG_NO_WINOGRAD_F43)) continue;
            if (I < wino_min_c(tile) || O < wino_min_c(tile)) continue;
            std::vector<float> U((size_t)(tile + 2) * (tile + 2) * O * I);
            wino_transform_weights(p.data(), O, I, U.data(), tile);
            (tile == 4 ? c.wino_u4 : c.wino_u2) = e->upload(U);
            if (tile == 4 && (e->cfg.flags & (IRSDE_FLAG_SPLIT_BF16X2 | IRSDE_FLAG_SPLIT_F16X2)) && I >= split_min_cin()) {
                unsigned short* up = nullptr;
                IRSDE_HIP_CHECK(hipMalloc(&up, U.size() * 4));
                e->dev_allocs.push_back(reinterpret_cast<float*>(up));
                const bool f16 = (e->cfg.flags & IRSDE_FLAG_SPLIT_F16X2) != 0;
                if (f16) c.wino_up_scale = pow2_scale_into_512(U.data(), U.size());
                launch_split_pairs(c.wino_u4, up, (size_t)36 * O, I, e->stream, f16, c.wino_up_scale);
                IRSDE_HIP_CHECK(hipStreamSynchronize(e->stream));
                c.wino_up = up;
            }
            if (tile == 4 && !(e->cfg.flags & IRSDE_FLAG_NO_WINOGRAD_FUSED) && O % 32 == 0 && I % 16 == 0 && I <= kWinoFusedMaxCin &&
                O <= kWinoFusedMaxCout) {
                std::vector<float> Uf(U.size());
                wino_fused_pack_weights(U.data(), O, I, Uf.data());
                c.wino_uf = e->upload(Uf);
            }
            if (tile == 4 && !(e->cfg.flags & IRSDE_FLAG_NO_WINOGRAD_FUSED) && wino_fused64_enabled() && O % 64 == 0 && I % 64 == 0 &&
                I <= wino_fused64_max_cin() && O <= wino_fused64_max_cout()) {
                std::vector<float> Uf(U.size());
                wino_fused64_pack_weights(U.data(), O, I, Uf.data());
                c.wino_uf64 = e->upload(Uf);
                if ((e->cfg.flags & IRSDE_FLAG_SPLIT_F16X2) && wino_fused64_pair_enabled()) {
                    c.wino_uf64p_scale = pow2_scale_into_512(U.data(), U.size());
                    unsigned short* up = nullptr;
                    IRSDE_HIP_CHECK(hipMalloc(&up, Uf.size() * 4));
                    e->dev_allocs.push_back(reinterpret_cast<float*>(up));
                    launch_wino_fused64_split_weights(c.wino_uf64, up, Uf.size(), c.wino_uf64p_scale, e->stream);
                    IRSDE_HIP_CHECK(hipStreamSynchronize(e->stream));
                    c.wino_uf64p = up;
                }
            }
        }
    }
    return c;
}

ConvW pack_init_conv(irsde_engine* e) {
    const HostTensor& t = need(e, "init_conv.weight");
    const int O = (int)t.shape[0], I = (int)t.shape[1];
    const int P = (I + 3) & ~3;
    const int CK = (7 * P + 31) & ~31;
    std::vector<float> p((size_t)O * 7 * CK, 0.f);
    for (int o = 0; o < O; ++o)
        for (int i = 0; i < I; ++i)
            for (int ky = 0; ky < 7; ++ky)
                for (int kx = 0; kx < 7; ++kx)
                    p[((size_t)o * 7 + ky) * CK + kx * P + i] = t.data[(((size_t)o * I + i) * 7 + ky) * 7 + kx];
    ConvW c;
    c.w = e->upload(p);
    c.Cout = O; c.Cin = CK; c.KH = 7; c.KW = 1;
    return c;
}

ResW pack_res(irsde_engine* e, const std::string& p) {
    ResW r;
    r.b1 = pack_conv(e, p + "block1.proj.weight", "");
    r.b2 = pack_conv(e, p + "block2.proj.weight", "");
    r.Cout = r.b1.Cout;
    r.has_res = e->host.count(p + "res_conv.weight") > 0;
    if (r.has_res) r.res = pack_conv(e, p + "res_conv.weight", "");
    r.mlp_w = e->upload(need(e, p + "mlp.1.weight").data);
    r.mlp_b = e->upload(need(e, p + "mlp.1.bias").data);
    return r;
}
AttnW pack_attn(irsde_engine* e, const std::string& p) {
    AttnW a;
    a.g1 = e->upload(need(e, p + "fn.norm.g").data);
    a.qkv = pack_conv(e, p + "fn.fn.to_qkv.weight", "");
    a.out = pack_conv(e, p + "fn.fn.to_out.0.weight", p + "fn.fn.to_out.0.bias");
    a.g2 = e->upload(need(e, p + "fn.fn.to_out.1.g").data);
    a.C = a.out.Cout;
    return a;
}

void inv_nafblock(irsde_engine* e, const std::string& p, int c) {
    const int td = e->time_dim;
    const std::string tm = naf_lens(e) ? "time_mlp.1." : "mlp.1.";
    add_w(e, p + tm + "weight", {4 * c, td / 2});
    add_w(e, p + tm + "bias", {4 * c});
    if (naf_lens(e)) {
        add_w(e, p + "cam_mlp.1.weight", {2 * c, td / 2});
        add_w(e, p + "cam_mlp.1.bias", {2 * c});
    }
    add_w(e, p + "conv1.weight", {2 * c, c, 1, 1});
    add_w(e, p + "conv1.bias", {2 * c});
    add_w(e, p + "conv2.weight", {2 * c, 1, 3, 3});
    add_w(e, p + "conv2.bias", {2 * c});
    add_w(e, p + "conv3.weight", {c, c, 1, 1});
    add_w(e, p + "conv3.bias", {c});
    add_w(e, p + "sca.1.weight", {c, c, 1, 1});
    add_w(e, p + "sca.1.bias", {c});
    add_w(e, p + "conv4.weight", {2 * c, c, 1, 1});
    add_w(e, p + "conv4.bias", {2 * c});
    add_w(e, p + "conv5.weight", {c, c, 1, 1});
    add_w(e, p + "conv5.bias", {c});
    add_w(e, p + "norm1.g", {1, c, 1, 1});
    add_w(e, p + "norm2.g", {1, c, 1, 1});
    add_w(e, p + "beta", {1, c, 1, 1});
    add_w(e, p + "gamma", {1, c, 1, 1});
    if (naf_stereo(e)) {
        const std::string f = p + "fusion.";
        add_w(e, f + "norm_l.g", {1, c, 1, 1});
        add_w(e, f + "norm_r.g", {1, c, 1, 1});
        for (const char* pr : {"l_proj1.", "r_proj1.", "l_proj2.", "r_proj2."}) {
            add_w(e, f + pr + "weight", {c, c, 1, 1});
            add_w(e, f + pr + "bias", {c});
        }
        add_w(e, f + "beta", {1, c, 1, 1});
        add_w(e, f + "gamma", {1, c, 1, 1});
    }
}
void build_inventory_naf(irsde_engine* e) {
    const int width = e->cfg.nf, ic = e->naf_ic, td = e->time_dim;
    const std::string t1 = naf_lens(e) ? "time_mlp.0." : "time_mlp.1.", t3 = naf_lens(e) ? "time_mlp.2." : "time_mlp.3.";
    add_w(e, t1 + "weight", {td * 2, width});
    add_w(e, t1 + "bias", {td * 2});
    add_w(e, t3 + "weight", {td, td});
    add_w(e, t3 + "bias", {td});
    if (naf_lens(e)) {
        add_w(e, "cam_mlp.0.weight", {td * 2, 3 * width});
        add_w(e, "cam_mlp.0.bias", {td * 2});
        add_w(e, "cam_mlp.2.weight", {td, td});
        add_w(e, "cam_mlp.2.bias", {td});
    }
    add_w(e, "intro.weight", {width, (uncond_engine(e) ? 1 : 2) * ic, 3, 3});
    add_w(e, "intro.bias", {width});
    add_w(e, "ending.weight", {ic, width, 3, 3});
    add_w(e, "ending.bias", {ic});
    int chan = width;
    for (size_t i = 0; i < e->naf_enc_nums.size(); ++i) {
        for (int j = 0; j < e->naf_enc_nums[i]; ++j)
            inv_nafblock(e, "encoders." + std::to_string(i) + "." + std::to_string(j) + ".", chan);
        add_w(e, "downs." + std::to_string(i) + ".weight", {2 * chan, chan, 2, 2});
        add_w(e, "downs." + std::to_string(i) + ".bias", {2 * chan});
        chan *= 2;
    }
// ... 295 lines not shown
    if (isum != I) throw HipError("pack_conv_pad: channel split mismatch for " + wname);
    const int Op = pad_out ? rup32(O) : O;
    std::vector<float> p((size_t)Op * KH * KW * Ip, 0.f);
    for (int o = 0; o < O; ++o) {
        int src = 0, dst = 0;
        for (int c : splits) {
            for (int i = 0; i < c; ++i)
                for (int ky = 0; ky < KH; ++ky)
                    for (int kx = 0; kx < KW; ++kx)
                        p[(((size_t)o * KH + ky) * KW + kx) * Ip + dst + i] = t.data[(((size_t)o * I + src + i) * KH + ky) * KW + kx];
            src += c;
            dst += rup32(c);
        }
    }
    ConvW cw;
    cw.w = e->upload(p);
    cw.Cout = Op; cw.Cin = Ip; cw.KH = KH; cw.KW = KW;
    if (!bname.empty()) {
        std::vector<float> pb(Op, 0.f);
        const HostTensor& b = need(e, bname);
        for (int o = 0; o < O; ++o) pb[o] = b.data[o];
        cw.bias = e->upload(pb);
    }
    return cw;
}

void finalize_latent(irsde_engine* e) {
    const int depth = (int)e->lat_mult.size(), ch = e->lat_ch;
    auto dim = [&](int i) { return i == 0 ? ch : ch * e->lat_mult[i - 1]; };
    auto resb = [&](const std::string& p, const std::vector<int>& in_splits, int co) {
        ResW r;
        r.b1 = pack_conv_pad(e, p + "block1.proj.weight", "", in_splits, true);
        r.b2 = pack_conv_pad(e, p + "block2.proj.weight", "", {co}, true);
        r.Cout = r.b1.Cout;
        r.has_res = e->host.count(p + "res_conv.weight") > 0;
        if (r.has_res) r.res = pack_conv_pad(e, p + "res_conv.weight", "", in_splits, true);
        return r;
    };
    e->lat_init = pack_conv_pad(e, "init_conv.weight", "", {e->lat_in}, true);
    e->lat_dec_res.resize(2 * depth);
    e->lat_up.resize(depth);
    for (int i = 0; i < depth; ++i) {
        const int di = dim(i), dout = dim(i + 1);
        const std::string en = "encoder." + std::to_string(i) + ".";
        e->lat_enc_res.push_back(resb(en + "0.", {di}, di));
        e->lat_enc_res.push_back(resb(en + "1.", {di}, di));
        if (i == depth - 1) {
            if (di % 32) throw HipError("latent UNet: the attention level needs a channel count that is a multiple of 32");
            e->lat_enc_attn = pack_attn(e, en + "2.");
        }
        e->lat_down.push_back(pack_conv_pad(e, en + "3.weight", i != depth - 1 ? en + "3.bias" : "", {di}, true));
        const int j = depth - 1 - i;
        const std::string de = "decoder." + std::to_string(j) + ".";
        e->lat_dec_res[2 * j] = resb(de + "0.", {dout, di}, dout);
        e->lat_dec_res[2 * j + 1] = resb(de + "1.", {dout, di}, dout);
        if (i == depth - 1) {
            if (dout % 32) throw HipError("latent UNet: the attention level needs a channel count that is a multiple of 32");
            e->lat_dec_attn = pack_attn(e, de + "2.");
        }
        e->lat_up[j] = i != 0 ? pack_conv_pad(e, de + "3.1.weight", de + "3.1.bias", {dout}, true)
                              : pack_conv_pad(e, de + "3.weight", "", {dout}, true);
    }
    e->lat_latent = pack_conv_pad(e, "latent_conv.weight", "", {dim(depth)}, true);
    e->lat_post = pack_conv_pad(e, "post_latent_conv.weight", "", {e->lat_embed}, true);
    e->lat_final = pack_conv_pad(e, "final_conv.weight", "final_conv.bias", {ch}, false);
}

void finalize(irsde_engine* e) {
    DeviceScope dev_scope(e->cfg.device);
    for (auto& n : e->names)
        if (!e->host[n].loaded) throw HipError("missing weight: " + n);
    if (e->arch == 2) {
        finalize_latent(e);
        finalize_common(e);
        return;
    }
    if (e->arch == 1) {
        finalize_naf(e);
        finalize_common(e);
        return;
    }
    const int depth = e->cfg.depth;
    e->init_conv = pack_init_conv(e);
    e->tm_w1 = e->upload(need(e, "time_mlp.1.weight").data);
    e->tm_b1 = e->upload(need(e, "time_mlp.1.bias").data);
    e->tm_w3 = e->upload(need(e, "time_mlp.3.weight").data);
    e->tm_b3 = e->upload(need(e, "time_mlp.3.bias").data);
    {
        const int half = e->cfg.nf / 2;
        std::vector<float> f(half);
        const double emb = std::log(10000.0) / (half - 1);
        for (int i = 0; i < half; ++i) f[i] = expf((float)i * (float)(-emb));
        e->freqs = e->upload(f);
    }
    e->down_res.reserve(2 * depth);
    e->up_res.reserve(2 * depth);
    for (int i = 0; i < depth; ++i) {
        const std::string d = "downs." + std::to_string(i) + ".";
        e->down_res.push_back(pack_res(e, d + "0."));
        e->down_res.push_back(pack_res(e, d + "1."));
        e->down_attn.push_back(pack_attn(e, d + "2."));
        e->down_conv.push_back(pack_conv(e, d + "3.weight", i != depth - 1 ? d + "3.bias" : ""));
    }
    e->mid1 = pack_res(e, "mid_block1.");
    if (e->cfg.flags & IRSDE_FLAG_UNCOND_FULLATTN) {
        AttnW a;
        a.g1 = e->upload(need(e, "mid_attn.fn.norm.g").data);
        a.qkv = pack_conv(e, "mid_attn.fn.fn.to_qkv.weight", "");
        a.out = pack_conv(e, "mid_attn.fn.fn.to_out.weight", "mid_attn.fn.fn.to_out.bias");
        a.C = a.out.Cout;
        e->mid_attn = a;
    } else {
        e->mid_attn = pack_attn(e, "mid_attn.");
    }
    e->mid2 = pack_res(e, "mid_block2.");
    for (int j = 0; j < depth; ++j) {
        const std::string u = "ups." + std::to_string(j) + ".";
        e->up_res.push_back(pack_res(e, u + "0."));
        e->up_res.push_back(pack_res(e, u + "1."));
        e->up_attn.push_back(pack_attn(e, u + "2."));
        if (j != depth - 1)
            e->up_conv.push_back(pack_conv(e, u + "3.1.weight", u + "3.1.bias"));
        else
            e->up_conv.push_back(pack_conv(e, u + "3.weight", ""));
    }
    e->final_res = pack_res(e, "final_res_block.");
    e->final_conv = pack_conv(e, "final_conv.weight", "final_conv.bias");

    e->all_res.clear();
    for (auto& r : e->down_res) e->all_res.push_back(&r);
    e->all_res.push_back(&e->mid1);
    e->all_res.push_back(&e->mid2);
    for (auto& r : e->up_res) e->all_res.push_back(&r);
    e->all_res.push_back(&e->final_res);
    int off = 0;
    for (ResW* r : e->all_res) {
        r->film_off = off;
        off += 2 * r->Cout;
    }
    e->film_row = off;
    finalize_common(e);
}

void finalize_common(irsde_engine* e) {
    conv_global_init();
    e->zeros = e->dmalloc(256);
    IRSDE_HIP_CHECK(hipMemset(e->zeros, 0, 1024));
    IRSDE_HIP_CHECK(hipStreamCreateWithFlags(&e->stream, hipStreamNonBlocking));
    IRSDE_HIP_CHECK(hipEventCreateWithFlags(&e->ev_in, hipEventDisableTiming));
    IRSDE_HIP_CHECK(hipEventCreateWithFlags(&e->ev_out, hipEventDisableTiming));
    e->step = reinterpret_cast<StepState*>(e->dmalloc(sizeof(StepState) / 4 + 4));
    e->ctl = reinterpret_cast<SampleCtl*>(e->dmalloc(sizeof(SampleCtl) / 4 + 4));
    IRSDE_HIP_CHECK(hipMemset(e->step, 0, sizeof(StepState)));
    IRSDE_HIP_CHECK(hipMemset(e->ctl, 0, sizeof(SampleCtl)));
    for (auto& kv : e->host) std::vector<float>().swap(kv.second.data);
    e->finalized = true;
}

void compute_film_rows(irsde_engine* e, const float* tvals, int rows, float* dst, hipStream_t s) {
    const int nf = e->cfg.nf, td = e->time_dim;
    float* emb = nullptr;
    float* h1 = nullptr;
    float* h2 = nullptr;
    IRSDE_HIP_CHECK(hipMalloc(&emb, (size_t)rows * nf * 4));
    IRSDE_HIP_CHECK(hipMalloc(&h1, (size_t)rows * td * 4));
    IRSDE_HIP_CHECK(hipMalloc(&h2, (size_t)rows * td * 4));
// ... 38 lines not shown
```

### image_restoration_sde_amd/csrc/kernels_misc.hip

```cpp
#include "common.h"
#include <algorithm>
#include <type_traits>

namespace irsde {

typedef float floatx16 __attribute__((ext_vector_type(16)));
typedef float floatx4 __attribute__((ext_vector_type(4)));
typedef __bf16 bf16_t;
typedef __bf16 bf16x4 __attribute__((ext_vector_type(4)));
typedef _Float16 f16x4 __attribute__((ext_vector_type(4)));
typedef _Float16 f16x8 __attribute__((ext_vector_type(8)));
typedef __bf16 bf16x8 __attribute__((ext_vector_type(8)));
typedef float floatx8 __attribute__((ext_vector_type(8)));

namespace {

template <bool F16OP>
struct Mf16 {
    using x8 = bf16x8;
    using x4 = bf16x4;
    static __device__ __forceinline__ floatx16 mfma(x8 a, x8 b, floatx16 c) { return __builtin_amdgcn_mfma_f32_32x32x16_bf16(a, b, c, 0, 0, 0); }
};
template <>
struct Mf16<true> {
// ... 1178 lines not shown

__global__ __launch_bounds__(256) void row_linear_kernel(const float* __restrict__ in, const int in_stride,
                                                         const float* __restrict__ W, const float* __restrict__ bias,
                                                         float* __restrict__ out, const int out_stride, const int rows,
                                                         const int in_dim, const int out_dim, const int act_in,
                                                         const int act_out) {
    const int lane = threadIdx.x & 63;
    const int o = blockIdx.x * 4 + (threadIdx.x >> 6);
    if (o >= out_dim) return;
    const float* w = W + (size_t)o * in_dim;
    const float bo = bias ? bias[o] : 0.f;
    for (int r = 0; r < rows; ++r) {
        const float* x = in + (size_t)r * in_stride;
        float s = 0.f;
        for (int i = lane; i < in_dim; i += 64) s = fmaf(act_apply(x[i], act_in), w[i], s);
        s = wave_xor_sum(s, 64);
        if (lane == 0) out[(size_t)r * out_stride + o] = act_apply(s + bo, act_out);
    }
}

__global__ __launch_bounds__(1024) void step_begin_kernel(StepState* st, const float* __restrict__ film_table, const int film_row,
                                                          float* __restrict__ film_cur, const float* __restrict__ coef_table) {
    const int t = st->t_next;
    __syncthreads();
    const float* src = film_table + (size_t)t * film_row;
    if ((film_row & 3) == 0 && ((reinterpret_cast<size_t>(src) | reinterpret_cast<size_t>(film_cur)) & 15) == 0) {
        const int n4 = film_row >> 2;
        const float4* s4 = reinterpret_cast<const float4*>(src);
        float4* d4 = reinterpret_cast<float4*>(film_cur);
        for (int i0 = threadIdx.x; i0 < n4; i0 += 8 * (int)blockDim.x) {
            float4 v[8];
#pragma unroll
            for (int j = 0; j < 8; ++j) {
                const int i = i0 + j * (int)blockDim.x;
                v[j] = s4[i < n4 ? i : i0];
            }
#pragma unroll
            for (int j = 0; j < 8; ++j) {
                const int i = i0 + j * (int)blockDim.x;
                if (i < n4) d4[i] = v[j];
            }
        }
    } else {
        for (int i = threadIdx.x; i < film_row; i += blockDim.x) film_cur[i] = src[i];
    }
    if (threadIdx.x < 12) st->coef[threadIdx.x] = coef_table[(size_t)t * 12 + threadIdx.x];
    if (threadIdx.x == 0) {
        st->t = t;
        st->t_next = t - 1;
    }
}

__global__ void set_step_kernel(StepState* st, const int t_next) {
    st->t = t_next;
    st->t_next = t_next;
}

__device__ __forceinline__ void philox4x32_10(uint32_t c0, uint32_t c1, uint32_t c2, uint32_t c3, uint32_t k0,
                                              uint32_t k1, uint32_t out[4]) {
#pragma unroll
    for (int r = 0; r < 10; ++r) {
        const uint32_t hi0 = __umulhi(0xD2511F53u, c0), lo0 = 0xD2511F53u * c0;
        const uint32_t hi1 = __umulhi(0xCD9E8D57u, c2), lo1 = 0xCD9E8D57u * c2;
        const uint32_t n0 = hi1 ^ c1 ^ k0, n2 = hi0 ^ c3 ^ k1;
        c0 = n0; c1 = lo1; c2 = n2; c3 = lo0;
        k0 += 0x9E3779B9u; k1 += 0xBB67AE85u;
    }
    out[0] = c0; out[1] = c1; out[2] = c2; out[3] = c3;
}

__device__ __forceinline__ void philox_normal4(uint32_t quad, uint32_t t, uint32_t image, uint64_t seed, float z[4]) {
    uint32_t r[4];
    philox4x32_10(quad, t, image, 0x1D5DEu, (uint32_t)seed, (uint32_t)(seed >> 32), r);
    const float s = 1.0f / 16777216.0f;
    const float u0 = ((float)(r[0] >> 8) + 0.5f) * s, u1 = ((float)(r[1] >> 8) + 0.5f) * s;
    const float u2 = ((float)(r[2] >> 8) + 0.5f) * s, u3 = ((float)(r[3] >> 8) + 0.5f) * s;
    const float ra = sqrtf(-2.0f * logf(u0)), rb = sqrtf(-2.0f * logf(u2));
    float sa, ca, sb, cb;
    sincosf(6.28318530717958647692f * u1, &sa, &ca);
    sincosf(6.28318530717958647692f * u3, &sb, &cb);
    z[0] = ra * ca; z[1] = ra * sa; z[2] = rb * cb; z[3] = rb * sb;
}

__global__ __launch_bounds__(256) void sde_update_kernel(const UpdateParams p) {
    const int b = blockIdx.y;
    const int CHW = p.C * p.H * p.W;
    const int HW = p.H * p.W;
    const int quad = blockIdx.x * blockDim.x + threadIdx.x;
    if (quad * 4 >= CHW) return;
    const int t = p.st ? p.st->t : p.t_imm;
    const float* cf = p.st ? p.st->coef : p.coef_imm;
    const float theta = cf[0], sigma = cf[1], sbar = cf[2], dt = cf[3];
    const float sqdt = cf[4], gain = cf[5], t1 = cf[6], t2 = cf[7];
    const float pstd = cf[8];
    int mode = p.mode;
    const float* noise = p.noise;
    long long noise_tstride = p.noise_tstride;
    unsigned long long seed = p.seed, image_offset = p.image_offset;
    if (p.ctl) {
        mode = p.ctl->mode; noise = p.ctl->noise; noise_tstride = p.ctl->noise_tstride;
        seed = p.ctl->seed; image_offset = p.ctl->image_offset;
    }
    float z[4] = {0.f, 0.f, 0.f, 0.f};
    const bool need_z = mode != 1 && mode != 4;
    const int bg = b + p.batch0;
    if (need_z && !noise) philox_normal4((uint32_t)quad, (uint32_t)t, (uint32_t)(image_offset + bg), seed, z);
    for (int k = 0; k < 4; ++k) {
        const int e = quad * 4 + k;
        if (e >= CHW) break;
        const size_t si = (size_t)b * CHW + e;
        const int c = e / HW, rem = e - c * HW, y = rem / p.W, xx = rem - y * p.W;
        const float eps_hat = p.pred[(size_t)b * p.sb + (size_t)c * p.sc + (size_t)y * p.sy + (size_t)xx * p.sx];
        const float x = p.x[si], mu = p.mu[si];
        if (need_z && noise) z[k] = noise[(size_t)t * noise_tstride + (size_t)bg * CHW + e];
        float xn;
        if (mode >= 3) {
            const float score = -eps_hat / sbar;
            if (mode == 3) {
                const float drift = -0.5f * (sigma * sigma) * (1.0f + cf[9]) * score * dt;
                const float disp = sigma * (z[k] * sqdt);
                xn = x - drift - disp;
            } else {
                const float drift = -0.5f * (sigma * sigma) * cf[9] * score * dt;
                xn = x - drift;
            }
        } else if (mode == 2) {
            const float x0 = (x - mu - sbar * eps_hat) * gain + mu;
            const float mean = t1 * (x - mu) + t2 * (x0 - mu) + mu;
            xn = mean + pstd * z[k];
        } else {
            const float score = -eps_hat / sbar;
            if (mode == 0) {
                const float drift = (theta * (mu - x) - sigma * sigma * score) * dt;
                const float disp = sigma * (z[k] * sqdt);
                xn = x - drift - disp;
            } else {
                const float drift = (theta * (mu - x) - 0.5f * (sigma * sigma) * score) * dt;
                xn = x - drift;
            }
        }
        p.x[si] = xn;
    }
}

__global__ void set_ctl_kernel(SampleCtl* ctl, const int mode, const float* noise, const long long noise_tstride,
                               const unsigned long long seed, const unsigned long long image_offset) {
    ctl->mode = mode; ctl->pad = 0; ctl->noise = noise; ctl->noise_tstride = noise_tstride;
    ctl->seed = seed; ctl->image_offset = image_offset;
}

__global__ void unpack_pred_kernel(const float* __restrict__ pred, float* __restrict__ out, const int B, const int C,
                                   const int H, const int W, const int Hp, const int Wp, const int stride) {
    const size_t idx = (size_t)blockIdx.x * blockDim.x + threadIdx.x;
    const size_t total = (size_t)B * C * H * W;
    if (idx >= total) return;
    const int x = (int)(idx % W);
    size_t r = idx / W;
    const int y = (int)(r % H); r /= H;
    const int c = (int)(r % C);
    const int b = (int)(r / C);
    out[idx] = pred[(((size_t)b * Hp + y) * Wp + x) * stride + c];
}

template <typename T>
__global__ void nhwc_to_nchw_kernel(const T* __restrict__ in, float* __restrict__ out, const int B, const int C,
                                    const int H, const int W) {
    const size_t idx = (size_t)blockIdx.x * blockDim.x + threadIdx.x;
    const size_t total = (size_t)B * C * H * W;
    if (idx >= total) return;
    const int x = (int)(idx % W);
    size_t r = idx / W;
    const int y = (int)(r % H); r /= H;
    const int c = (int)(r % C);
    const int b = (int)(r / C);
    out[idx] = ld1(in + (((size_t)b * H + y) * W + x) * C + c);
}

constexpr int kDwRows = 4;
constexpr int kDwRun = 16;

struct DwGeom {
    int gpp, PP, run, tiles_x, tiles_y;
};
static inline DwGeom dw_geom(int H, int W, int c) {
    DwGeom g;
    const int G = c >> 2;
    g.gpp = G < 256 ? G : 256;
    g.PP = 256 / g.gpp;
    g.run = (W + g.PP - 1) / g.PP;
    g.run = g.run < 4 ? 4 : g.run > kDwRun ? kDwRun : g.run;
    g.tiles_x = (W + g.PP * g.run - 1) / (g.PP * g.run);
    g.tiles_y = (H + kDwRows - 1) / kDwRows;
    return g;
}

__global__ __launch_bounds__(256) void dwconv_gate_kernel(const float* __restrict__ u, const float* __restrict__ w,
                                                          const float* __restrict__ bias, float* __restrict__ out,
                                                          float* __restrict__ partial, const int H, const int W,
                                                          const int c, const int tiles_x, const int ntiles, const int run) {
    __shared__ float4 red[256];
    constexpr int R = kDwRows;
    const int tile = blockIdx.x, b = blockIdx.y;
    const int ty = tile / tiles_x, tx = tile - ty * tiles_x;
    const int HW = H * W;
    const int G = c >> 2;
    const int gpp = G < 256 ? G : 256;
    const int PP = 256 / gpp;
    const int C2 = 2 * c;
    for (int gc = 0; gc < G; gc += gpp) {
        const int g = gc + (int)(threadIdx.x % gpp);
        const int pl = threadIdx.x / gpp;
        float4 sum = make_float4(0.f, 0.f, 0.f, 0.f);
        const int y0 = ty * R, x0 = (tx * PP + pl) * run;
        if (g < G && pl < PP && x0 < W) {
            const int ch = g * 4;
            const float4 b1 = *reinterpret_cast<const float4*>(bias + ch);
            const float4 b2 = *reinterpret_cast<const float4*>(bias + c + ch);
            float4 w1[9], w2[9];
#pragma unroll
            for (int k = 0; k < 9; ++k) {
                w1[k] = *reinterpret_cast<const float4*>(w + k * C2 + ch);
                w2[k] = *reinterpret_cast<const float4*>(w + k * C2 + c + ch);
            }
            const float4 zero = make_float4(0.f, 0.f, 0.f, 0.f);
// ... 501 lines not shown
    if (wq_pair && wout_pair) {
        const size_t planes_x = (size_t)2 * 128 * (2 * C + 16), planes_o = (size_t)2 * 128 * (2 * kHid + 16);
        const size_t ys = (size_t)128 * ((C > kHid ? C : kHid) + 4) * sizeof(float);
        const size_t ldsp = std::max(std::max(planes_x, planes_o), ys);
        const dim3 gridp((N + 127) / 128, B);
        if (C == 64)
            hipLaunchKernelGGL((attn_q_out_fused_kernel<64, true>), gridp, dim3(256), ldsp, s, xn, x, wq, ws.ctx, wout, bias, g2, y, N, eps, ln_g,
                               wq_pair, wout_pair, wq_inv, wout_inv);
        else if (C == 128)
            hipLaunchKernelGGL((attn_q_out_fused_kernel<128, true>), gridp, dim3(256), ldsp, s, xn, x, wq, ws.ctx, wout, bias, g2, y, N, eps, ln_g,
                               wq_pair, wout_pair, wq_inv, wout_inv);
        else
            hipLaunchKernelGGL((attn_q_out_fused_kernel<256, true>), gridp, dim3(256), ldsp, s, xn, x, wq, ws.ctx, wout, bias, g2, y, N, eps, ln_g,
                               wq_pair, wout_pair, wq_inv, wout_inv);
        IRSDE_HIP_CHECK(hipGetLastError());
        return;
    }
    const size_t lds = (size_t)128 * ((C > kHid ? C : kHid) + 4) * sizeof(float);
    const dim3 grid((N + 127) / 128, B);
    if (C == 64)
        hipLaunchKernelGGL(attn_q_out_fused_kernel<64>, grid, dim3(256), lds, s, xn, x, wq, ws.ctx, wout, bias, g2, y, N, eps, ln_g);
    else if (C == 128)
        hipLaunchKernelGGL(attn_q_out_fused_kernel<128>, grid, dim3(256), lds, s, xn, x, wq, ws.ctx, wout, bias, g2, y, N, eps, ln_g);
    else
        hipLaunchKernelGGL(attn_q_out_fused_kernel<256>, grid, dim3(256), lds, s, xn, x, wq, ws.ctx, wout, bias, g2, y, N, eps, ln_g);
    IRSDE_HIP_CHECK(hipGetLastError());
}

void launch_linear_attention(const float* qkv, float* out, int B, int N, const AttnWorkspace& ws, hipStream_t s, bool bf16) {
    if (bf16)
        linear_attention_t(reinterpret_cast<const bf16_t*>(qkv), reinterpret_cast<bf16_t*>(out), B, N, ws, s);
    else
        linear_attention_t(qkv, out, B, N, ws, s);
}

void launch_full_attention(const float* qkv, float* out, int B, int N, hipStream_t s) {
    const int qtiles = (N + 31) / 32;
    hipLaunchKernelGGL(full_attn_kernel, dim3((qtiles + 3) / 4, B * kHeads), dim3(256), 0, s, qkv, out, N,
                       1.0f / sqrtf((float)kDh));
    IRSDE_HIP_CHECK(hipGetLastError());
}

void launch_prep_input(const float* xt, const float* cond, float* x0, int B, int in_nc, int H, int W, int Hp, int Wp,
                       hipStream_t s, int reflect) {
    const int P = ((cond ? 2 : 1) * in_nc + 3) & ~3;
    if (P > 16) throw HipError("prep_input: more than 8 (conditional) / 16 (unconditional) input channels unsupported");
    const size_t total = (size_t)B * (Hp + 6) * (Wp + 6);
    hipLaunchKernelGGL(prep_input_kernel, dim3((unsigned)((total + 255) / 256)), dim3(256), 0, s, xt, cond, x0, B,
                       in_nc, P, H, W, Hp, Wp, reflect);
    IRSDE_HIP_CHECK(hipGetLastError());
}

void launch_sinusoid(const float* tvals, const float* freqs, float* out, int rows, int half, hipStream_t s) {
    const int total = rows * half;
    hipLaunchKernelGGL(sinusoid_kernel, dim3((total + 255) / 256), dim3(256), 0, s, tvals, freqs, out, rows, half);
    IRSDE_HIP_CHECK(hipGetLastError());
}

void launch_row_linear(const float* in, int in_stride, const float* W, const float* b, float* out, int out_stride,
                       int rows, int in_dim, int out_dim, int act_in, int act_out, hipStream_t s) {
    hipLaunchKernelGGL(row_linear_kernel, dim3((out_dim + 3) / 4), dim3(256), 0, s, in, in_stride, W, b, out,
                       out_stride, rows, in_dim, out_dim, act_in, act_out);
    IRSDE_HIP_CHECK(hipGetLastError());
}

void launch_step_begin(StepState* st, const float* film_table, int film_row, float* film_cur, const float* coef_table,
                       hipStream_t s) {
    hipLaunchKernelGGL(step_begin_kernel, dim3(1), dim3(1024), 0, s, st, film_table, film_row, film_cur, coef_table);
    IRSDE_HIP_CHECK(hipGetLastError());
}

void launch_set_step(StepState* st, int t_next, hipStream_t s) {
    hipLaunchKernelGGL(set_step_kernel, dim3(1), dim3(1), 0, s, st, t_next);
    IRSDE_HIP_CHECK(hipGetLastError());
}

void launch_sde_update(const UpdateParams& p, hipStream_t s) {
    const int CHW = p.C * p.H * p.W;
    const int quads = (CHW + 3) / 4;
    hipLaunchKernelGGL(sde_update_kernel, dim3((quads + 255) / 256, p.B), dim3(256), 0, s, p);
    IRSDE_HIP_CHECK(hipGetLastError());
}

void launch_set_ctl(SampleCtl* ctl, int mode, const float* noise, long long noise_tstride, unsigned long long seed,
                    unsigned long long image_offset, hipStream_t s) {
    hipLaunchKernelGGL(set_ctl_kernel, dim3(1), dim3(1), 0, s, ctl, mode, noise, noise_tstride, seed, image_offset);
    IRSDE_HIP_CHECK(hipGetLastError());
}

void launch_unpack_pred(const float* pred, float* out, int B, int C, int H, int W, int Hp, int Wp, int stride, hipStream_t s) {
    const size_t total = (size_t)B * C * H * W;
    hipLaunchKernelGGL(unpack_pred_kernel, dim3((unsigned)((total + 255) / 256)), dim3(256), 0, s, pred, out, B, C, H,
                       W, Hp, Wp, stride);
    IRSDE_HIP_CHECK(hipGetLastError());
}

void launch_nhwc_to_nchw(const float* in, float* out, int B, int C, int H, int W, hipStream_t s, bool bf16) {
    const size_t total = (size_t)B * C * H * W;
    if (bf16)
        hipLaunchKernelGGL(nhwc_to_nchw_kernel<bf16_t>, dim3((unsigned)((total + 255) / 256)), dim3(256), 0, s,
                           reinterpret_cast<const bf16_t*>(in), out, B, C, H, W);
    else
        hipLaunchKernelGGL(nhwc_to_nchw_kernel<float>, dim3((unsigned)((total + 255) / 256)), dim3(256), 0, s, in, out, B, C, H,
                           W);
    IRSDE_HIP_CHECK(hipGetLastError());
}

void launch_fill_random(float* p, size_t n, unsigned seed, float scale, hipStream_t s) {
    const size_t quads = (n + 3) / 4;
    hipLaunchKernelGGL(fill_random_kernel, dim3((unsigned)((quads + 255) / 256)), dim3(256), 0, s, p, n, seed, scale);
    IRSDE_HIP_CHECK(hipGetLastError());
}

void launch_philox_normal(float* out, int B, int CHW, int t, uint64_t seed, uint64_t image_offset, hipStream_t s) {
    const int quads = (CHW + 3) / 4;
    hipLaunchKernelGGL(philox_normal_kernel, dim3((quads + 255) / 256, B), dim3(256), 0, s, out, CHW, t, seed,
                       image_offset);
    IRSDE_HIP_CHECK(hipGetLastError());
}

__global__ void bf16_to_f32_kernel(const bf16_t* __restrict__ in, float* __restrict__ out, size_t n) {
    const size_t i = (size_t)blockIdx.x * blockDim.x + threadIdx.x;
    if (i < n) out[i] = (float)in[i];
}
void launch_bf16_to_f32(const unsigned short* in, float* out, size_t n, hipStream_t s) {
    hipLaunchKernelGGL(bf16_to_f32_kernel, dim3((unsigned)((n + 255) / 256)), dim3(256), 0, s, reinterpret_cast<const bf16_t*>(in), out, n);
    IRSDE_HIP_CHECK(hipGetLastError());
}

__global__ void add_kernel(const float* __restrict__ a, const float* __restrict__ b, float* __restrict__ out, size_t n4) {
    const size_t i = (size_t)blockIdx.x * blockDim.x + threadIdx.x;
    if (i >= n4) return;
    const float4 x = reinterpret_cast<const float4*>(a)[i], y = reinterpret_cast<const float4*>(b)[i];
    reinterpret_cast<float4*>(out)[i] = make_float4(x.x + y.x, x.y + y.y, x.z + y.z, x.w + y.w);
}
void launch_add(const float* a, const float* b, float* out, size_t n, hipStream_t s) {
    if (n % 4) throw HipError("launch_add: element count must be a multiple of 4");
    hipLaunchKernelGGL(add_kernel, dim3((unsigned)((n / 4 + 255) / 256)), dim3(256), 0, s, a, b, out, n / 4);
    IRSDE_HIP_CHECK(hipGetLastError());
}

__global__ void nchw_to_nhwc_pad_kernel(const float* __restrict__ in, float* __restrict__ out, const int B, const int C,
                                        const int H, const int W, const int Hp, const int Wp, const int Cp, const int reflect) {
    const size_t idx = (size_t)blockIdx.x * blockDim.x + threadIdx.x;
    const size_t total = (size_t)B * Hp * Wp * Cp;
    if (idx >= total) return;
    const int c = (int)(idx % Cp);
    size_t r = idx / Cp;
    const int x = (int)(r % Wp); r /= Wp;
    const int y = (int)(r % Hp);
    const int b = (int)(r / Hp);
    float v = 0.f;
    if (c < C && (reflect || (y < H && x < W))) {
        const int sy = y < H ? y : 2 * (H - 1) - y, sx = x < W ? x : 2 * (W - 1) - x;
        v = in[(((size_t)b * C + c) * H + sy) * W + sx];
    }
    out[idx] = v;
}
void launch_nchw_to_nhwc_pad(const float* in, float* out, int B, int C, int H, int W, int Hp, int Wp, int Cp, int reflect,
                             hipStream_t s) {
    const size_t total = (size_t)B * Hp * Wp * Cp;
    hipLaunchKernelGGL(nchw_to_nhwc_pad_kernel, dim3((unsigned)((total + 255) / 256)), dim3(256), 0, s, in, out, B, C, H, W, Hp,
                       Wp, Cp, reflect);
    IRSDE_HIP_CHECK(hipGetLastError());
}

// ... 24 lines not shown
```

### include/irsde_hip.h

```cpp
#ifndef IRSDE_HIP_H
#define IRSDE_HIP_H

#include <stdint.h>

#ifdef __cplusplus
extern "C" {
#endif

typedef struct irsde_engine irsde_engine;

enum {
    IRSDE_OK = 0,
    IRSDE_ERR_INVALID = -1,
    IRSDE_ERR_HIP = -2,
    IRSDE_ERR_STATE = -3,
    IRSDE_ERR_WEIGHT = -4
};

enum { IRSDE_MODE_SDE = 0, IRSDE_MODE_ODE = 1, IRSDE_MODE_POSTERIOR = 2,
       IRSDE_MODE_DSDE_SDE = 3, IRSDE_MODE_DSDE_ODE = 4 };

enum {
    IRSDE_FLAG_KEEP_ACTIVATIONS = 1,
    IRSDE_FLAG_NAIVE_CONV = 2,
    IRSDE_FLAG_NO_WINOGRAD = 4,
    IRSDE_FLAG_UNCOND_FULLATTN = 16,
    IRSDE_FLAG_BF16 = 32,
    IRSDE_FLAG_BF16_ACT = 128,
    IRSDE_FLAG_NO_FUSED_LN = 256,
    IRSDE_FLAG_NAF_LENS = 512,
    IRSDE_FLAG_NAF_INTRO_SKIP = 64,
    IRSDE_FLAG_FP16 = 1024,
    IRSDE_FLAG_NO_WINOGRAD_FUSED = 2048,
    IRSDE_FLAG_NO_FUSED_ATTN = 4096,
    IRSDE_FLAG_SPLIT_BF16X2 = 16384,
    IRSDE_FLAG_SPLIT_F16X2 = 32768,
    IRSDE_FLAG_NO_NAF_CHAIN = 8192,
    IRSDE_FLAG_NAF_STEREO = 65536,
    IRSDE_FLAG_NAF_UNCOND = 131072,
    IRSDE_FLAG_NO_WINOGRAD_F43 = 8
};
enum {
    IRSDE_SAMPLE_GRAPH = 1,
    IRSDE_SAMPLE_PROFILE = 2
};

typedef struct irsde_config {
    int32_t in_nc;
    int32_t out_nc;
    int32_t nf;
    int32_t depth;
    int32_t device;
    int32_t flags;
} irsde_config;

typedef struct irsde_nafnet_config {
    int32_t img_channel;
    int32_t width;
    int32_t middle_blk_num;
    int32_t n_enc;
    int32_t enc_blk_nums[8];
    int32_t n_dec;
    int32_t dec_blk_nums[8];
    int32_t device;
    int32_t flags;
} irsde_nafnet_config;

typedef struct irsde_latent_unet_config {
    int32_t in_ch;
    int32_t out_ch;
    int32_t ch;
    int32_t n_mult;
    int32_t ch_mult[8];
    int32_t embed_dim;
    int32_t device;
    int32_t flags;
} irsde_latent_unet_config;

#define IRSDE_COEF_STRIDE 12

const char* irsde_last_error(void);
int irsde_version(void);

int irsde_create(const irsde_config* cfg, irsde_engine** out);
int irsde_create_nafnet(const irsde_nafnet_config* cfg, irsde_engine** out);
void irsde_destroy(irsde_engine* e);

int irsde_num_weights(const irsde_engine* e);
const char* irsde_weight_name(const irsde_engine* e, int index);
int irsde_weight_shape(const irsde_engine* e, int index, int64_t shape[4], int* ndim);

int irsde_load_weight(irsde_engine* e, const char* name, const float* data, const int64_t* shape, int ndim);
int irsde_finalize_weights(irsde_engine* e);

int irsde_set_schedule(irsde_engine* e, int T, const float* coef);

int irsde_unet_forward(irsde_engine* e, const float* xt, const float* cond, const int64_t* t_host, int nt, int B,
                       int H, int W, float* out, void* stream);

int irsde_sample(irsde_engine* e, int mode, const float* xT, const float* mu, const float* noise, uint64_t seed,
                 uint64_t image_offset, int B, int H, int W, int T, int t_stop, float* out, void* stream,
                 int flags);

int irsde_sde_step(int mode, int t, const float* coef_row, float* x, const float* mu, const float* eps_hat,
                   const float* noise_t, uint64_t seed, uint64_t image_offset, int B, int C, int H, int W,
                   void* stream);

int irsde_philox_normal(float* out, int B, int CHW, int t, uint64_t seed, uint64_t image_offset, void* stream);

int irsde_get_profile(const irsde_engine* e, double out[12]);

int irsde_debug_tap(irsde_engine* e, const char* name, float* dst, int64_t dims[4]);

int irsde_work_model(irsde_engine* e, int B, int H, int W, double out[2]);

int irsde_op_profile(irsde_engine* e, char* buf, int buflen);

int irsde_plan_describe(irsde_engine* e, int B, int H, int W, char* buf, int buflen);

int irsde_create_latent_unet(const irsde_latent_unet_config* cfg, irsde_engine** out);
int irsde_latent_shapes(irsde_engine* e, int H, int W, int64_t latent_chw[3], int64_t* hidden_chw, int* n_hidden);
int irsde_latent_encode(irsde_engine* e, const float* x, int B, int H, int W, float* latent, float* const* hidden,
// ... 17 lines not shown
```

### include/irsde_hip_debug.h

```cpp
#ifndef IRSDE_HIP_DEBUG_H
#define IRSDE_HIP_DEBUG_H

#include "irsde_hip.h"

#ifdef __cplusplus
extern "C" {
#endif

int irsde_debug_conv(const float* in0, int C0, const float* in1, int C1, int B, int Hin, int Win, int in_shift,
                     const float* w_oihw, int Cout, int KH, int KW, int stride, int pad, const float* bias,
                     const float* film, int film_bstride, int silu, const float* res, float* out, int naive,
                     int splits, void* stream);

int irsde_debug_split_gemm(const float* A, const float* B, float* C, int M, int N, int K, int ncomp, int nplanes, void* stream);

int irsde_bench_conv(int variant, int B, int H, int W, int Cin, int Cout, int K, int stride, int up, int epi, int iters,
                     double* ms_out);
int irsde_bench_naf_chain(int variant, int nblocks, int B, int iters, double* ms_out);
int irsde_debug_force_subbatches(int n);
int irsde_debug_force_chain_groups(int g);

int irsde_debug_scam(const float* x, int B_pairs, int H, int W, int C, const float* norm_l_g, const float* norm_r_g, const float* l_proj1_w,
                     const float* l_proj1_b, const float* r_proj1_w, const float* r_proj1_b, const float* l_proj2_w, const float* l_proj2_b,
                     const float* r_proj2_w, const float* r_proj2_b, const float* beta, const float* gamma, float* out, void* stream);

#ifdef __cplusplus
}
#endif
#endif
```

Before: 4.265 images/s.

## Hoist condition half of init conv per call and fuse final conv with SDE update

The init 7x1 conv is split into an x part and a cond part. The cond contribution is computed once per sampler call instead of at every step, since mu does not change across steps. The final 64->3 channel 3x3 conv is fused with the SDE update into a single tiled kernel that holds eps in shared memory and writes x directly. This removes a pred round-trip and one launch per step, at the cost of a separate step op list, new flags, and more complex plan bookkeeping.

```diff
diff --git a/image_restoration_sde_amd/_lib.py b/image_restoration_sde_amd/_lib.py
--- a/image_restoration_sde_amd/_lib.py
+++ b/image_restoration_sde_amd/_lib.py
@@ -27,6 +27,8 @@
 FLAG_SPLIT_F16X2 = 32768
 FLAG_NAF_STEREO = 65536
 FLAG_NAF_UNCOND = 131072
+FLAG_NO_COND_HOIST = 262144
+FLAG_NO_FINAL_STEP = 524288
 SAMPLE_GRAPH = 1
 SAMPLE_PROFILE = 2
 
@@ -34,7 +36,7 @@
     "irsde_last_error", "irsde_version", "irsde_create", "irsde_create_nafnet", "irsde_destroy", "irsde_num_weights",
     "irsde_weight_name", "irsde_weight_shape", "irsde_load_weight", "irsde_finalize_weights",
     "irsde_set_schedule", "irsde_unet_forward", "irsde_sample", "irsde_sde_step", "irsde_philox_normal",
-    "irsde_get_profile", "irsde_debug_tap", "irsde_work_model", "irsde_debug_conv", "irsde_plan_describe", "irsde_bench_conv", "irsde_op_profile", "irsde_debug_split_gemm", "irsde_bench_naf_chain", "irsde_debug_force_subbatches", "irsde_debug_force_chain_groups", "irsde_debug_scam",
+    "irsde_get_profile", "irsde_debug_tap", "irsde_work_model", "irsde_debug_conv", "irsde_plan_describe", "irsde_bench_conv", "irsde_op_profile", "irsde_debug_split_gemm", "irsde_bench_naf_chain", "irsde_debug_force_subbatches", "irsde_debug_force_chain_groups", "irsde_debug_scam", "irsde_debug_final_step",
     "irsde_eval_metrics", "irsde_tensor2img",
     "irsde_set_lens_info", "irsde_create_latent_unet", "irsde_latent_shapes", "irsde_latent_encode", "irsde_latent_decode", "irsde_latent_hidden",
 ]
@@ -119,6 +121,7 @@
     lib.irsde_debug_force_subbatches.argtypes = [c.c_int]
     lib.irsde_debug_force_chain_groups.argtypes = [c.c_int]
     lib.irsde_debug_scam.argtypes = [P, c.c_int, c.c_int, c.c_int, c.c_int] + [P] * 12 + [P, P]
+    lib.irsde_debug_final_step.argtypes = [c.c_int, c.c_int, c.c_int, P, P, P, P, P, P, P, c.c_uint64, c.c_uint64] + [c.c_int] * 6 + [P, P]
     lib.irsde_debug_split_gemm.argtypes = [P, P, P, c.c_int, c.c_int, c.c_int, c.c_int, c.c_int, P]
     lib.irsde_eval_metrics.argtypes = [P, P, c.c_int, c.c_int, c.c_int, c.c_int, c.c_int, c.POINTER(c.c_double), P]
     lib.irsde_tensor2img.argtypes = [P, P, c.c_int, c.c_int, c.c_int, c.c_int, P]
diff --git a/image_restoration_sde_amd/csrc/common.h b/image_restoration_sde_amd/csrc/common.h
--- a/image_restoration_sde_amd/csrc/common.h
+++ b/image_restoration_sde_amd/csrc/common.h
@@ -156,6 +156,7 @@
 
 double conv_flops(const ConvParams& p);
 void launch_conv(const ConvParams& p, hipStream_t s);
+void launch_conv_narrow(const ConvParams& p, hipStream_t s);
 void conv_global_init();
 void conv_halo_global_init();
 bool conv_halo_eligible(const ConvParams& p);
@@ -273,6 +274,17 @@
     int batch0;
 };
 void launch_sde_update(const UpdateParams& p, hipStream_t s);
+struct FinalStepParams {
+    const float* in = nullptr;
+    const float* w = nullptr;
+    const float* bias = nullptr;
+    int Cout = 0, Hp = 0, Wp = 0;
+    float* pred = nullptr;
+    int pred_stride = 0;
+    UpdateParams u;
+};
+bool final_step_ok(int Cin, int Cout, int C);
+void launch_final_step(const FinalStepParams& p, hipStream_t s);
 void launch_philox_normal(float* out, int B, int CHW, int t, uint64_t seed, uint64_t image_offset, hipStream_t s);
 
 void eval_metrics(const float* out, const float* gt, int B, int C, int H, int W, int crop, double* sums_host, hipStream_t s);
diff --git a/image_restoration_sde_amd/csrc/conv_igemm.hip b/image_restoration_sde_amd/csrc/conv_igemm.hip
--- a/image_restoration_sde_amd/csrc/conv_igemm.hip
+++ b/image_restoration_sde_amd/csrc/conv_igemm.hip
@@ -1233,6 +1233,15 @@
     return bn;
 }
 
+void launch_conv_narrow(const ConvParams& p, hipStream_t s) {
+    const int M = p.B * p.Ho * p.Wo;
+    if (p.w_bf || p.Cout > 3 || p.C0 != 64 || p.C1 || p.KH != 3 || p.KW != 3 || p.stride != 1 || p.pad_y != 1 || p.pad_x != 1 || p.in_shift || p.film || p.silu ||
+        p.res || p.splits != 1 || p.nz != 1 || !p.zeros)
+        throw HipError("launch_conv_narrow: a plain 64 -> 1..3 channel 3x3 s1 p1 layer only");
+    hipLaunchKernelGGL(conv3x3_narrow_kernel, dim3((M + 16 * kNarrowPPG - 1) / (16 * kNarrowPPG)), dim3(256), 0, s, p, M);
+    IRSDE_HIP_CHECK(hipGetLastError());
+}
+
 void launch_conv(const ConvParams& p, hipStream_t s) {
     const int M = p.B * p.Ho * p.Wo;
     const int Ctot = p.C0 + p.C1;
@@ -1270,8 +1279,7 @@
     if (!p.w_bf && g_variant == 0 && p.Cout <= 3 && p.C0 == 64 && p.KH == 3 && p.KW == 3 && p.stride == 1 && p.pad_y == 1 && p.pad_x == 1 &&
         !p.in_shift && !p.C1 && !p.film && !p.silu && !p.res && p.splits == 1 && p.nz == 1 && !p.gate && !p.shuffle &&
         !p.ch_scale && !p.in_scale && !p.ln_g && M >= 65536) {
-        hipLaunchKernelGGL(conv3x3_narrow_kernel, dim3((M + 16 * kNarrowPPG - 1) / (16 * kNarrowPPG)), dim3(256), 0, s, p, M);
-        IRSDE_HIP_CHECK(hipGetLastError());
+        launch_conv_narrow(p, s);
         return;
     }
     if (const int zb = zloop_batch(p)) {
diff --git a/image_restoration_sde_amd/csrc/engine.h b/image_restoration_sde_amd/csrc/engine.h
--- a/image_restoration_sde_amd/csrc/engine.h
+++ b/image_restoration_sde_amd/csrc/engine.h
@@ -206,6 +206,11 @@
     int slot = 0, b0 = 0;
     std::vector<PoolBlock> pool;
     std::vector<Op> net_ops;
+    std::vector<Op> call_ops, step_ops;
+    bool step_has_update = false;
+    float* x0s = nullptr;
+    float* cond_c = nullptr;
+    double step_conv_flops = 0, step_conv_bytes = 0, step_conv_exec_flops = 0;
     float* xin = nullptr;
     float* cin = nullptr;
     float* x0 = nullptr;
@@ -276,6 +281,7 @@
     std::vector<float*> dev_allocs;
 
     ConvW init_conv, final_conv;
+    ConvW init_conv_x, init_conv_c;
     float *tm_w1 = nullptr, *tm_b1 = nullptr, *tm_w3 = nullptr, *tm_b3 = nullptr, *freqs = nullptr;
     std::vector<ResW> down_res;
     std::vector<AttnW> down_attn;
@@ -417,6 +423,7 @@
 int forced_chain_groups();
 void set_force_subbatches(int n);
 LatentPlan* get_latent_plan(irsde_engine* e, int B, int H, int W, bool decode);
+UpdateParams make_update(irsde_engine* e, Plan* pl);
 
 int guard(const std::function<void()>& f);
 
diff --git a/image_restoration_sde_amd/csrc/engine_api.hip b/image_restoration_sde_amd/csrc/engine_api.hip
--- a/image_restoration_sde_amd/csrc/engine_api.hip
+++ b/image_restoration_sde_amd/csrc/engine_api.hip
@@ -21,21 +21,12 @@
     for (auto& op : pl->net_ops) op.fn(s);
 }
 
-UpdateParams make_update(irsde_engine* e, Plan* pl) {
-    UpdateParams u{};
-    u.x = pl->xin; u.mu = pl->cin; u.pred = pl->pred;
-    const int64_t ps = pl->pred_stride;
-    u.sb = (int64_t)pl->Hp * pl->Wp * ps; u.sc = 1; u.sy = (int64_t)pl->Wp * ps; u.sx = ps;
-    u.st = step_of(e, pl); u.ctl = e->ctl;
-    u.B = pl->B; u.C = e->cfg.in_nc; u.H = pl->H; u.W = pl->W;
-    u.batch0 = pl->b0;
-    return u;
-}
+const std::vector<Op>& step_ops_of(const Plan* pl) { return pl->step_ops.empty() ? pl->net_ops : pl->step_ops; }
 
 void one_step(irsde_engine* e, Plan* pl, hipStream_t s) {
     launch_step_begin(step_of(e, pl), e->film_table, e->film_row, film_of(e, pl), e->coef_table, s);
-    run_net(pl, s);
-    launch_sde_update(make_update(e, pl), s);
+    for (auto& op : step_ops_of(pl)) op.fn(s);
+    if (!pl->step_has_update) launch_sde_update(make_update(e, pl), s);
 }
 
 void ensure_step_graph(irsde_engine* e, Plan* pl, hipStream_t s) {
@@ -354,6 +345,7 @@
             IRSDE_HIP_CHECK(hipMemcpyAsync(pl->xin, xT + i * simg, simg * 4, hipMemcpyDeviceToDevice, t));
             if (mu) IRSDE_HIP_CHECK(hipMemcpyAsync(pl->cin, mu + i * simg, simg * 4, hipMemcpyDeviceToDevice, t));
             launch_set_step(step_of(e, pl), T, t);
+            for (auto& op : pl->call_ops) op.fn(t);
             if (graph) ensure_step_graph(e, pl, t);
         }
         if (!profile) {
@@ -364,6 +356,7 @@
                 }
         } else {
             Plan* pl = parts[0].pl;
+            const std::vector<Op>& ops = step_ops_of(pl);
             std::vector<int> kinds;
             size_t ei = 0;
             auto mark = [&](int kind) {
@@ -373,20 +366,20 @@
             for (int i = 0; i < nsteps; ++i) {
                 mark(OP_OTHER);
                 launch_step_begin(step_of(e, pl), e->film_table, e->film_row, film_of(e, pl), e->coef_table, s);
-                for (auto& op : pl->net_ops) {
+                for (auto& op : ops) {
                     mark(op.kind);
                     op.fn(s);
                 }
                 mark(OP_OTHER);
-                launch_sde_update(make_update(e, pl), s);
+                if (!pl->step_has_update) launch_sde_update(make_update(e, pl), s);
             }
             IRSDE_HIP_CHECK(hipEventRecord(get_event(e, ei++), s));
             IRSDE_HIP_CHECK(hipStreamSynchronize(s));
             double ms[OP_NKINDS] = {0, 0, 0, 0, 0};
-            const size_t per_step = pl->net_ops.size() + 2;
-            e->op_ms.assign(pl->net_ops.size(), 0.0);
+            const size_t per_step = ops.size() + 2;
+            e->op_ms.assign(ops.size(), 0.0);
             e->op_desc.clear();
-            for (auto& op : pl->net_ops) e->op_desc.push_back(op.desc);
+            for (auto& op : ops) e->op_desc.push_back(op.desc);
             e->op_steps = nsteps;
             e->op_split = naf_subbatches(e, B, H, W);
             for (size_t k = 0; k < kinds.size(); ++k) {
@@ -394,24 +387,25 @@
                 IRSDE_HIP_CHECK(hipEventElapsedTime(&t, e->ev_pool[k], e->ev_pool[k + 1]));
                 ms[kinds[k]] += t;
                 const size_t in_step = k % per_step;
-                if (in_step >= 1 && in_step <= pl->net_ops.size()) e->op_ms[in_step - 1] += t;
+                if (in_step >= 1 && in_step <= ops.size()) e->op_ms[in_step - 1] += t;
             }
             hipEvent_t e0 = e->ev_pool[0], e1 = e->ev_pool[kinds.size()];
             float wall;
             IRSDE_HIP_CHECK(hipEventElapsedTime(&wall, e0, e1));
             size_t nconv = 0;
-            for (auto& op : pl->net_ops) nconv += op.kind == OP_CONV;
+            for (auto& op : ops) nconv += op.kind == OP_CONV;
+            const bool spec = !pl->step_ops.empty();
             e->profile[0] = ms[OP_CONV];
-            e->profile[1] = pl->conv_flops * nsteps;
+            e->profile[1] = (spec ? pl->step_conv_flops : pl->conv_flops) * nsteps;
             e->profile[2] = (double)nconv * nsteps;
-            e->profile[3] = pl->conv_bytes * nsteps;
+            e->profile[3] = (spec ? pl->step_conv_bytes : pl->conv_bytes) * nsteps;
             e->profile[4] = ms[OP_LN];
             e->profile[5] = ms[OP_ATTN];
             e->profile[6] = ms[OP_OTHER];
             e->profile[7] = wall;
             e->profile[8] = nsteps;
             e->profile[9] = ms[OP_WINO];
-            e->profile[10] = pl->conv_exec_flops * nsteps;
+            e->profile[10] = (spec ? pl->step_conv_exec_flops : pl->conv_exec_flops) * nsteps;
             e->profile[11] = 0;
         }
         for (int i = 0; i < nsub; ++i) {
@@ -508,6 +502,13 @@
         Plan* pl = get_plan(e, B, H, W, false);
         std::string out;
         for (auto& op : pl->net_ops) out += op.desc + "\n";
+        for (auto& op : pl->call_ops) out += "sampler per call: " + op.desc + "\n";
+        if (!pl->step_ops.empty()) {
+            const size_t ns = pl->step_ops.size();
+            for (size_t i = 0; i < 2 && i < ns; ++i)
+                if (pl->step_ops[i].desc != pl->net_ops[i].desc) out += "sampler step: " + pl->step_ops[i].desc + "\n";
+            if (pl->step_has_update) out += "sampler step: " + pl->step_ops[ns - 1].desc + "\n";
+        }
         const int nsub = naf_subbatches(e, B, H, W);
         if (nsub > 1) out += "note: the un-split plan; irsde_sample runs this batch as " + std::to_string(nsub) + " concurrent sub-batches of " + std::to_string(B / nsub) + " images (own plans)\n";
         strncpy(buf, out.c_str(), buflen - 1);
@@ -522,8 +523,8 @@
         std::lock_guard<std::mutex> lk(e->mu);
         DeviceScope dev_scope(e->cfg.device);
         Plan* pl = get_plan(e, B, H, W, false);
-        out[0] = pl->conv_flops;
-        out[1] = pl->conv_bytes;
+        out[0] = pl->step_ops.empty() ? pl->conv_flops : pl->step_conv_flops;
+        out[1] = pl->step_ops.empty() ? pl->conv_bytes : pl->step_conv_bytes;
     });
 }
 
diff --git a/image_restoration_sde_amd/csrc/engine_debug.hip b/image_restoration_sde_amd/csrc/engine_debug.hip
--- a/image_restoration_sde_amd/csrc/engine_debug.hip
+++ b/image_restoration_sde_amd/csrc/engine_debug.hip
@@ -124,6 +124,51 @@
         }
         launch_scam_core(qv, F, B, H, W, C, s);
         launch_scam_epilogue(x, F, dbe, dga, out, B, H, W, C, s);
+        IRSDE_HIP_CHECK(hipStreamSynchronize(s));
+    });
+}
+
+int irsde_debug_final_step(int fused, int mode, int t, const float* coef_row, const float* feat, const float* w_oihw, const float* bias, float* x,
+                           const float* mu, const float* noise_t, uint64_t seed, uint64_t image_offset, int B, int C, int H, int W, int Hp, int Wp,
+                           float* eps_out, void* stream) {
+    return guard([&] {
+        if (!coef_row || !feat || !w_oihw || !x || !mu) throw HipError("null argument");
+        if (mode < 0 || mode > 2) throw HipError("debug_final_step: bad mode");
+        if (B < 1 || H < 1 || W < 1 || Hp < H || Wp < W || !final_step_ok(64, C, C)) throw HipError("debug_final_step: bad shape");
+        hipStream_t s = reinterpret_cast<hipStream_t>(stream);
+        Scratch mem(s);
+        std::vector<float> wp((size_t)C * 9 * 64);
+        for (int o = 0; o < C; ++o)
+            for (int i = 0; i < 64; ++i)
+                for (int k = 0; k < 9; ++k) wp[((size_t)o * 9 + k) * 64 + i] = w_oihw[((size_t)o * 64 + i) * 9 + k];
+        float* dw = mem.upload(wp);
+        float* db = bias ? mem.upload(bias, C) : nullptr;
+        float* dz = mem.alloc<float>(256);
+        IRSDE_HIP_CHECK(hipMemset(dz, 0, 1024));
+        UpdateParams u{};
+        u.x = x; u.mu = mu;
+        u.noise = noise_t; u.noise_tstride = 0;
+        u.st = nullptr; u.ctl = nullptr; u.t_imm = t;
+        for (int i = 0; i < IRSDE_COEF_STRIDE; ++i) u.coef_imm[i] = coef_row[i];
+        u.mode = mode; u.B = B; u.C = C; u.H = H; u.W = W; u.seed = seed; u.image_offset = image_offset;
+        if (fused) {
+            FinalStepParams fp;
+            fp.in = feat; fp.w = dw; fp.bias = db; fp.Cout = C; fp.Hp = Hp; fp.Wp = Wp;
+            fp.pred = eps_out; fp.pred_stride = 4;
+            fp.u = u;
+            launch_final_step(fp, s);
+        } else {
+            float* pred = eps_out ? eps_out : mem.alloc<float>((size_t)B * Hp * Wp * 4);
+            ConvParams p;
+            p.in0 = feat; p.C0 = 64; p.pix0 = 64; p.Hin = Hp; p.Win = Wp;
+            p.w = dw; p.Cout = C; p.KH = p.KW = 3; p.stride = 1; p.pad_y = p.pad_x = 1;
+            p.B = B; p.Ho = Hp; p.Wo = Wp;
+            p.out = pred; p.out_stride = 4; p.bias = db; p.zeros = dz;
+            launch_conv_narrow(p, s);
+            u.pred = pred;
+            u.sb = (int64_t)Hp * Wp * 4; u.sc = 1; u.sy = (int64_t)Wp * 4; u.sx = 4;
+            launch_sde_update(u, s);
+        }
         IRSDE_HIP_CHECK(hipStreamSynchronize(s));
     });
 }
diff --git a/image_restoration_sde_amd/csrc/engine_plan.hip b/image_restoration_sde_amd/csrc/engine_plan.hip
--- a/image_restoration_sde_amd/csrc/engine_plan.hip
+++ b/image_restoration_sde_amd/csrc/engine_plan.hip
@@ -895,19 +895,59 @@
         e->plans.push_back(std::move(plan));
         return pl;
     }
-    Tensor x;
+    const bool samp_fp32 = !uncond && !per_sample_film && !b.naive &&
+                           !(e->cfg.flags & (IRSDE_FLAG_BF16 | IRSDE_FLAG_BF16_ACT | IRSDE_FLAG_FP16 | IRSDE_FLAG_SPLIT_BF16X2 | IRSDE_FLAG_SPLIT_F16X2));
+    const bool hoist = samp_fp32 && !(e->cfg.flags & IRSDE_FLAG_NO_COND_HOIST) && e->init_conv_x.w && e->init_conv_c.w;
+    const bool fuse_final = samp_fp32 && !(e->cfg.flags & IRSDE_FLAG_NO_FINAL_STEP) && final_step_ok(e->final_conv.Cin, e->final_conv.Cout, in_nc);
+    Tensor x = b.talloc(B, pl->Hp, pl->Wp, nf);
+    auto init_conv_op = [&](const ConvW& cw, const float* src, int Pc, float* out, const float* res, int real_c) {
+        ConvParams p;
+        p.in0 = src; p.C0 = cw.Cin; p.pix0 = Pc;
+        p.Hin = pl->Hp + 6; p.Win = pl->Wp + 6;
+        p.w = cw.w; p.Cout = nf; p.KH = 7; p.KW = 1; p.stride = 1; p.pad_y = 0; p.pad_x = 0;
+        p.B = B; p.Ho = pl->Hp; p.Wo = pl->Wp;
+        p.out = out; p.out_stride = nf; p.out_bf16 = x.bf16;
+        if (res) { p.res = res; p.res_stride = nf; }
+        b.push_conv(p);
+        Op op = std::move(pl->net_ops.back());
+        pl->net_ops.pop_back();
+        pl->conv_flops -= op.flops; pl->conv_exec_flops -= op.exec_flops; pl->conv_bytes -= op.bytes;
+        op.flops = 2.0 * (double)B * pl->Hp * pl->Wp * nf * 49.0 * real_c;
+        return op;
+    };
+    auto count = [&](const Op& op, double sign) {
+        pl->conv_flops += sign * op.flops; pl->conv_exec_flops += sign * op.exec_flops; pl->conv_bytes += sign * op.bytes;
+    };
     {
-        ConvParams p;
-        p.in0 = pl->x0; p.C0 = e->init_conv.Cin; p.pix0 = P;
-        p.Hin = pl->Hp + 6; p.Win = pl->Wp + 6;
-        p.w = e->init_conv.w; p.Cout = nf; p.KH = 7; p.KW = 1; p.stride = 1; p.pad_y = 0; p.pad_x = 0;
-        p.B = B; p.Ho = pl->Hp; p.Wo = pl->Wp;
-        x = b.talloc(B, pl->Hp, pl->Wp, nf);
-        p.out = x.p; p.out_stride = nf; p.out_bf16 = x.bf16;
-        b.push_conv(p);
-        const double real = 2.0 * (double)B * pl->Hp * pl->Wp * nf * 49.0 * ((uncond ? 1.0 : 2.0) * in_nc);
-        pl->conv_flops += real - pl->net_ops.back().flops;
-        pl->net_ops.back().flops = real;
+        Op op = init_conv_op(e->init_conv, pl->x0, P, x.p, nullptr, (uncond ? 1 : 2) * in_nc);
+        count(op, 1.0);
+        pl->net_ops.push_back(std::move(op));
+    }
+    const size_t n_head = pl->net_ops.size();
+    Op head_prep, head_conv;
+    if (hoist) {
+        const int Ps = (in_nc + 3) & ~3;
+        const size_t x0n = (size_t)B * (pl->Hp + 6) * (pl->Wp + 6) * Ps + 64;
+        pl->x0s = pl->alloc(x0n, false);
+        IRSDE_HIP_CHECK(hipMemset(pl->x0s, 0, x0n * sizeof(float)));
+        pl->cond_c = pl->alloc((size_t)B * pl->Hp * pl->Wp * nf, false);
+        const float *xi = pl->xin, *ci = pl->cin;
+        float* x0s = pl->x0s;
+        const int Hp = pl->Hp, Wp = pl->Wp;
+        Op prep_mu;
+        prep_mu.kind = OP_OTHER;
+        prep_mu.desc = "prep(mu alone, 4 channels)";
+        prep_mu.fn = [=](hipStream_t s) { launch_prep_input(ci, nullptr, x0s, B, in_nc, H, W, Hp, Wp, s, 1); };
+        pl->call_ops.push_back(std::move(prep_mu));
+        Op cc = init_conv_op(e->init_conv_c, pl->x0s, Ps, pl->cond_c, nullptr, in_nc);
+        cc.desc = "condition " + cc.desc;
+        pl->call_ops.push_back(std::move(cc));
+        head_prep.kind = OP_OTHER;
+        head_prep.desc = "prep(x alone, 4 channels)";
+        head_prep.fn = [=](hipStream_t s) { launch_prep_input(xi, nullptr, x0s, B, in_nc, H, W, Hp, Wp, s, 1); };
+        head_conv = init_conv_op(e->init_conv_x, pl->x0s, Ps, x.p, pl->cond_c, in_nc);
+        head_conv.desc = "init " + head_conv.desc + " + condition tensor";
+        head_conv.bytes += 4.0 * (double)B * pl->Hp * pl->Wp * nf;
     }
     b.tap("init_conv", x);
     Tensor x_init = x;
@@ -968,9 +1008,54 @@
         Tensor pr = b.conv(e->final_conv, f, nullptr, 1, 1, 0, nullptr, 0, nullptr, pl->pred_stride);
         b.tfree(f);
         pl->pred = pr.p;
+        if (hoist || fuse_final) {
+            pl->step_conv_flops = pl->conv_flops; pl->step_conv_exec_flops = pl->conv_exec_flops; pl->step_conv_bytes = pl->conv_bytes;
+            auto swap_counts = [&](const Op& out, const Op& in) {
+                pl->step_conv_flops += in.flops - out.flops; pl->step_conv_exec_flops += in.exec_flops - out.exec_flops; pl->step_conv_bytes += in.bytes - out.bytes;
+            };
+            if (hoist) {
+                swap_counts(pl->net_ops[n_head - 1], head_conv);
+                pl->step_ops.push_back(std::move(head_prep));
+                pl->step_ops.push_back(std::move(head_conv));
+            } else {
+                for (size_t i = 0; i < n_head; ++i) pl->step_ops.push_back(pl->net_ops[i]);
+            }
+            const size_t n_mid = pl->net_ops.size() - (fuse_final ? 1 : 0);
+            for (size_t i = n_head; i < n_mid; ++i) pl->step_ops.push_back(pl->net_ops[i]);
+            if (fuse_final) {
+                FinalStepParams fp;
+                fp.in = f.p; fp.w = e->final_conv.w; fp.bias = e->final_conv.bias;
+                fp.Cout = e->final_conv.Cout; fp.Hp = pl->Hp; fp.Wp = pl->Wp;
+                fp.u = make_update(e, pl);
+                const Op& fc = pl->net_ops.back();
+                Op op;
+                op.kind = OP_CONV;
+                op.flops = fc.flops; op.exec_flops = fc.exec_flops;
+                op.bytes = fc.bytes - 4.0 * (double)B * pl->Hp * pl->Wp * pl->pred_stride;
+                char buf[200];
+                snprintf(buf, sizeof buf, "final conv 3x3 + reverse step (one launch) M=%d Cout=%d Cin=%d tiles=%lld flops=%.4g", B * pl->Hp * pl->Wp, fp.Cout, e->final_conv.Cin,
+                         (long long)B * ((pl->Hp + 7) / 8) * ((pl->Wp + 15) / 16), op.flops);
+                op.desc = buf;
+                op.fn = [fp](hipStream_t s) { launch_final_step(fp, s); };
+                swap_counts(fc, op);
+                pl->step_ops.push_back(std::move(op));
+                pl->step_has_update = true;
+            }
+        }
     }
     e->plans.push_back(std::move(plan));
     return pl;
+}
+
+UpdateParams make_update(irsde_engine* e, Plan* pl) {
+    UpdateParams u{};
+    u.x = pl->xin; u.mu = pl->cin; u.pred = pl->pred;
+    const int64_t ps = pl->pred_stride;
+    u.sb = (int64_t)pl->Hp * pl->Wp * ps; u.sc = 1; u.sy = (int64_t)pl->Wp * ps; u.sx = ps;
+    u.st = step_of(e, pl); u.ctl = e->ctl;
+    u.B = pl->B; u.C = e->cfg.in_nc; u.H = pl->H; u.W = pl->W;
+    u.batch0 = pl->b0;
+    return u;
 }
 
 LatentPlan* get_latent_plan(irsde_engine* e, int B, int H, int W, bool decode) {
diff --git a/image_restoration_sde_amd/csrc/engine_weights.hip b/image_restoration_sde_amd/csrc/engine_weights.hip
--- a/image_restoration_sde_amd/csrc/engine_weights.hip
+++ b/image_restoration_sde_amd/csrc/engine_weights.hip
@@ -153,6 +153,25 @@
     return c;
 }
 
+ConvW pack_init_conv_half(irsde_engine* e, int which) {
+    const HostTensor& t = need(e, "init_conv.weight");
+    const int O = (int)t.shape[0], I = (int)t.shape[1], Ih = I / 2;
+    const int P = (Ih + 3) & ~3;
+    const int CK = (7 * P + 31) & ~31;
+    std::vector<float> p((size_t)O * 7 * CK, 0.f);
+    for (int o = 0; o < O; ++o)
+        for (int i = 0; i < Ih; ++i)
+            for (int ky = 0; ky < 7; ++ky)
+                for (int kx = 0; kx < 7; ++kx) {
+                    const float wa = t.data[(((size_t)o * I + i) * 7 + ky) * 7 + kx], wb = t.data[(((size_t)o * I + Ih + i) * 7 + ky) * 7 + kx];
+                    p[((size_t)o * 7 + ky) * CK + kx * P + i] = which ? wb - wa : wa;
+                }
+    ConvW c;
+    c.w = e->upload(p);
+    c.Cout = O; c.Cin = CK; c.KH = 7; c.KW = 1;
+    return c;
+}
+
 ResW pack_res(irsde_engine* e, const std::string& p) {
     ResW r;
     r.b1 = pack_conv(e, p + "block1.proj.weight", "");
@@ -614,6 +633,10 @@
     }
     const int depth = e->cfg.depth;
     e->init_conv = pack_init_conv(e);
+    if (!uncond_engine(e)) {
+        e->init_conv_x = pack_init_conv_half(e, 0);
+        e->init_conv_c = pack_init_conv_half(e, 1);
+    }
     e->tm_w1 = e->upload(need(e, "time_mlp.1.weight").data);
     e->tm_b1 = e->upload(need(e, "time_mlp.1.bias").data);
     e->tm_w3 = e->upload(need(e, "time_mlp.3.weight").data);
diff --git a/image_restoration_sde_amd/csrc/kernels_misc.hip b/image_restoration_sde_amd/csrc/kernels_misc.hip
--- a/image_restoration_sde_amd/csrc/kernels_misc.hip
+++ b/image_restoration_sde_amd/csrc/kernels_misc.hip
@@ -1284,6 +1284,43 @@
     z[0] = ra * ca; z[1] = ra * sa; z[2] = rb * cb; z[3] = rb * sb;
 }
 
+struct UpdateCoef {
+    float theta, sigma, sbar, dt, sqdt, gain, t1, t2, pstd, c9;
+};
+__device__ __forceinline__ UpdateCoef load_update_coef(const float* cf) {
+    return UpdateCoef{cf[0], cf[1], cf[2], cf[3], cf[4], cf[5], cf[6], cf[7], cf[8], cf[9]};
+}
+__device__ __forceinline__ float sde_update_value(const int mode, const UpdateCoef& k, const float x, const float mu, const float eps_hat, const float z) {
+    const float theta = k.theta, sigma = k.sigma, sbar = k.sbar, dt = k.dt, sqdt = k.sqdt, gain = k.gain, t1 = k.t1, t2 = k.t2, pstd = k.pstd;
+    float xn;
+    if (mode >= 3) {
+        const float score = -eps_hat / sbar;
+        if (mode == 3) {
+            const float drift = -0.5f * (sigma * sigma) * (1.0f + k.c9) * score * dt;
+            const float disp = sigma * (z * sqdt);
+            xn = x - drift - disp;
+        } else {
+            const float drift = -0.5f * (sigma * sigma) * k.c9 * score * dt;
+            xn = x - drift;
+        }
+    } else if (mode == 2) {
+        const float x0 = (x - mu - sbar * eps_hat) * gain + mu;
+        const float mean = t1 * (x - mu) + t2 * (x0 - mu) + mu;
+        xn = mean + pstd * z;
+    } else {
+        const float score = -eps_hat / sbar;
+        if (mode == 0) {
+            const float drift = (theta * (mu - x) - sigma * sigma * score) * dt;
+            const float disp = sigma * (z * sqdt);
+            xn = x - drift - disp;
+        } else {
+            const float drift = (theta * (mu - x) - 0.5f * (sigma * sigma) * score) * dt;
+            xn = x - drift;
+        }
+    }
+    return xn;
+}
+
 __global__ __launch_bounds__(256) void sde_update_kernel(const UpdateParams p) {
     const int b = blockIdx.y;
     const int CHW = p.C * p.H * p.W;
@@ -1291,10 +1328,7 @@
     const int quad = blockIdx.x * blockDim.x + threadIdx.x;
     if (quad * 4 >= CHW) return;
     const int t = p.st ? p.st->t : p.t_imm;
-    const float* cf = p.st ? p.st->coef : p.coef_imm;
-    const float theta = cf[0], sigma = cf[1], sbar = cf[2], dt = cf[3];
-    const float sqdt = cf[4], gain = cf[5], t1 = cf[6], t2 = cf[7];
-    const float pstd = cf[8];
+    const UpdateCoef cf = load_update_coef(p.st ? p.st->coef : p.coef_imm);
     int mode = p.mode;
     const float* noise = p.noise;
     long long noise_tstride = p.noise_tstride;
@@ -1315,33 +1349,123 @@
         const float eps_hat = p.pred[(size_t)b * p.sb + (size_t)c * p.sc + (size_t)y * p.sy + (size_t)xx * p.sx];
         const float x = p.x[si], mu = p.mu[si];
         if (need_z && noise) z[k] = noise[(size_t)t * noise_tstride + (size_t)bg * CHW + e];
-        float xn;
-        if (mode >= 3) {
-            const float score = -eps_hat / sbar;
-            if (mode == 3) {
-                const float drift = -0.5f * (sigma * sigma) * (1.0f + cf[9]) * score * dt;
-                const float disp = sigma * (z[k] * sqdt);
-                xn = x - drift - disp;
-            } else {
-                const float drift = -0.5f * (sigma * sigma) * cf[9] * score * dt;
-                xn = x - drift;
-            }
-        } else if (mode == 2) {
-            const float x0 = (x - mu - sbar * eps_hat) * gain + mu;
-            const float mean = t1 * (x - mu) + t2 * (x0 - mu) + mu;
-            xn = mean + pstd * z[k];
-        } else {
-            const float score = -eps_hat / sbar;
-            if (mode == 0) {
-                const float drift = (theta * (mu - x) - sigma * sigma * score) * dt;
-                const float disp = sigma * (z[k] * sqdt);
-                xn = x - drift - disp;
-            } else {
-                const float drift = (theta * (mu - x) - 0.5f * (sigma * sigma) * score) * dt;
-                xn = x - drift;
-            }
-        }
-        p.x[si] = xn;
+        p.x[si] = sde_update_value(mode, cf, x, mu, eps_hat, z[k]);
+    }
+}
+
+constexpr int kFsTH = 8, kFsTW = 16, kFsPH = kFsTH + 2, kFsPW = kFsTW + 2;
+constexpr int kFsQuads = kFsTW / 4 + 1;
+__global__ __launch_bounds__(256) void final_step_kernel(const FinalStepParams p) {
+    __shared__ float4 tile[kFsPH * kFsPW * 16];
+    __shared__ float eps[3][kFsTH][kFsTW];
+    const int tid = threadIdx.x, l = tid & 15, g = tid >> 4;
+    int wgid;
+    {
+        const int orig = blockIdx.x, nwg = gridDim.x;
+        const int xcd = orig & 7, q = nwg >> 3, r = nwg & 7;
+        wgid = (xcd < r ? xcd * (q + 1) : r * (q + 1) + (xcd - r) * q) + (orig >> 3);
+    }
+    const int tiles_x = (p.Wp + kFsTW - 1) / kFsTW, tiles_y = (p.Hp + kFsTH - 1) / kFsTH;
+    const int tx = wgid % tiles_x, t1 = wgid / tiles_x, ty = t1 % tiles_y, b = t1 / tiles_y;
+    const int x0 = tx * kFsTW, y0 = ty * kFsTH;
+    float4 w[3][9];
+#pragma unroll
+    for (int co = 0; co < 3; ++co)
+#pragma unroll
+        for (int t = 0; t < 9; ++t)
+            w[co][t] = co < p.Cout ? *reinterpret_cast<const float4*>(p.w + ((size_t)co * 9 + t) * 64 + l * 4) : make_float4(0.f, 0.f, 0.f, 0.f);
+    {
+        constexpr int kN = (kFsPH * kFsPW * 16 + 255) / 256;
+        float4 v[kN];
+#pragma unroll
+        for (int i = 0; i < kN; ++i) {
+            const int idx = tid + i * 256, pix = idx >> 4;
+            const int py = pix / kFsPW, px = pix - py * kFsPW;
+            const int iy = y0 - 1 + py, ix = x0 - 1 + px;
+            const bool in = pix < kFsPH * kFsPW && (unsigned)iy < (unsigned)p.Hp && (unsigned)ix < (unsigned)p.Wp;
+            v[i] = in ? *reinterpret_cast<const float4*>(p.in + ((size_t)(b * p.Hp + iy) * p.Wp + ix) * 64 + l * 4) : make_float4(0.f, 0.f, 0.f, 0.f);
+        }
+#pragma unroll
+        for (int i = 0; i < kN; ++i) {
+            const int idx = tid + i * 256;
+            if (idx < kFsPH * kFsPW * 16) tile[idx] = v[i];
+        }
+    }
+    __syncthreads();
+    {
+        const int r = g >> 1, c0 = (g & 1) * 8;
+        float4 win[3][3];
+#pragma unroll
+        for (int ky = 0; ky < 3; ++ky) {
+            win[ky][1] = tile[((r + ky) * kFsPW + c0) * 16 + l];
+            win[ky][2] = tile[((r + ky) * kFsPW + c0 + 1) * 16 + l];
+        }
+#pragma unroll
+        for (int i = 0; i < 8; ++i) {
+#pragma unroll
+            for (int ky = 0; ky < 3; ++ky) {
+                win[ky][0] = win[ky][1];
+                win[ky][1] = win[ky][2];
+                win[ky][2] = tile[((r + ky) * kFsPW + c0 + i + 2) * 16 + l];
+            }
+            float acc[3] = {0.f, 0.f, 0.f};
+#pragma unroll
+            for (int ky = 0; ky < 3; ++ky)
+#pragma unroll
+                for (int kx = 0; kx < 3; ++kx) {
+                    const float4 v = win[ky][kx];
+#pragma unroll
+                    for (int co = 0; co < 3; ++co) {
+                        const float4 wv = w[co][ky * 3 + kx];
+                        acc[co] = fmaf(v.x, wv.x, acc[co]);
+                        acc[co] = fmaf(v.y, wv.y, acc[co]);
+                        acc[co] = fmaf(v.z, wv.z, acc[co]);
+                        acc[co] = fmaf(v.w, wv.w, acc[co]);
+                    }
+                }
+#pragma unroll
+            for (int o = 8; o > 0; o >>= 1)
+#pragma unroll
+                for (int co = 0; co < 3; ++co) acc[co] += __shfl_xor(acc[co], o, 64);
+            if (l < p.Cout) {
+                const float ev = (l == 0 ? acc[0] : l == 1 ? acc[1] : acc[2]) + (p.bias ? p.bias[l] : 0.f);
+                eps[l][r][c0 + i] = ev;
+                const int oy = y0 + r, ox = x0 + c0 + i;
+                if (p.pred && oy < p.Hp && ox < p.Wp) p.pred[((size_t)(b * p.Hp + oy) * p.Wp + ox) * p.pred_stride + l] = ev;
+            }
+        }
+    }
+    __syncthreads();
+    const UpdateParams& u = p.u;
+    const int slot = tid % kFsQuads, ry = (tid / kFsQuads) % kFsTH, c = tid / (kFsQuads * kFsTH);
+    const int y = y0 + ry;
+    if (c >= u.C || y >= u.H || x0 >= u.W) return;
+    const int CHW = u.C * u.H * u.W, HW = u.H * u.W;
+    const int ea = c * HW + y * u.W + x0, eb = ea + min(kFsTW, u.W - x0);
+    const int quad = (ea >> 2) + slot;
+    if (quad * 4 >= eb) return;
+    const int t = u.st ? u.st->t : u.t_imm;
+    const UpdateCoef cf = load_update_coef(u.st ? u.st->coef : u.coef_imm);
+    int mode = u.mode;
+    const float* noise = u.noise;
+    long long noise_tstride = u.noise_tstride;
+    unsigned long long seed = u.seed, image_offset = u.image_offset;
+    if (u.ctl) {
+        mode = u.ctl->mode; noise = u.ctl->noise; noise_tstride = u.ctl->noise_tstride;
+        seed = u.ctl->seed; image_offset = u.ctl->image_offset;
+    }
+    float z[4] = {0.f, 0.f, 0.f, 0.f};
+    const bool need_z = mode != 1 && mode != 4;
+    const int bg = b + u.batch0;
+    if (need_z && !noise) philox_normal4((uint32_t)quad, (uint32_t)t, (uint32_t)(image_offset + bg), seed, z);
+    for (int k = 0; k < 4; ++k) {
+        const int e = quad * 4 + k;
+        if (e < ea || e >= eb) continue;
+        const size_t si = (size_t)b * CHW + e;
+        const float eps_hat = eps[c][ry][e - ea];
+        const float x = u.x[si], mu = u.mu[si];
+        if (need_z && noise) z[k] = noise[(size_t)t * noise_tstride + (size_t)bg * CHW + e];
+        u.x[si] = sde_update_value(mode, cf, x, mu, eps_hat, z[k]);
     }
 }
 
@@ -2009,6 +2133,14 @@
     IRSDE_HIP_CHECK(hipGetLastError());
 }
 
+bool final_step_ok(int Cin, int Cout, int C) { return Cin == 64 && Cout >= 1 && Cout <= 3 && C == Cout; }
+void launch_final_step(const FinalStepParams& p, hipStream_t s) {
+    if (!final_step_ok(64, p.Cout, p.u.C) || p.u.H > p.Hp || p.u.W > p.Wp) throw HipError("final_step: needs a 64 -> 1..3 channel layer and a state of as many channels inside the padded map");
+    const long long tiles = (long long)p.u.B * ((p.Hp + kFsTH - 1) / kFsTH) * ((p.Wp + kFsTW - 1) / kFsTW);
+    hipLaunchKernelGGL(final_step_kernel, dim3((unsigned)tiles), dim3(256), 0, s, p);
+    IRSDE_HIP_CHECK(hipGetLastError());
+}
+
 void launch_set_ctl(SampleCtl* ctl, int mode, const float* noise, long long noise_tstride, unsigned long long seed,
                     unsigned long long image_offset, hipStream_t s) {
     hipLaunchKernelGGL(set_ctl_kernel, dim3(1), dim3(1), 0, s, ctl, mode, noise, noise_tstride, seed, image_offset);
diff --git a/include/irsde_hip.h b/include/irsde_hip.h
--- a/include/irsde_hip.h
+++ b/include/irsde_hip.h
@@ -38,6 +38,8 @@
     IRSDE_FLAG_NO_NAF_CHAIN = 8192,
     IRSDE_FLAG_NAF_STEREO = 65536,
     IRSDE_FLAG_NAF_UNCOND = 131072,
+    IRSDE_FLAG_NO_COND_HOIST = 262144,
+    IRSDE_FLAG_NO_FINAL_STEP = 524288,
     IRSDE_FLAG_NO_WINOGRAD_F43 = 8
 };
 enum {
diff --git a/include/irsde_hip_debug.h b/include/irsde_hip_debug.h
--- a/include/irsde_hip_debug.h
+++ b/include/irsde_hip_debug.h
@@ -24,6 +24,10 @@
                      const float* l_proj1_b, const float* r_proj1_w, const float* r_proj1_b, const float* l_proj2_w, const float* l_proj2_b,
                      const float* r_proj2_w, const float* r_proj2_b, const float* beta, const float* gamma, float* out, void* stream);
 
+int irsde_debug_final_step(int fused, int mode, int t, const float* coef_row, const float* feat, const float* w_oihw, const float* bias, float* x,
+                           const float* mu, const float* noise_t, uint64_t seed, uint64_t image_offset, int B, int C, int H, int W, int Hp, int Wp,
+                           float* eps_out, void* stream);
+
 #ifdef __cplusplus
 }
 #endif
```

Measured after the change: 4.292 images/s, median of 6. No clear change (+0.6%).
